# ThomasZiegler/RS-aware-differential-SfM

Hardware: AMD Instinct MI355X
Metric: Mpixels/sec RS depth+pose solve, 1280x720 pair (higher is better)
Workload: dtype f64

## Files before the change

### include/rsdsfm.h

```cpp
#ifndef RSDSFM_H
#define RSDSFM_H

#include <stddef.h>
#include <stdint.h>

#ifdef __cplusplus
extern "C" {
#endif

#define RSDSFM_OK 0
#define RSDSFM_ERR_INVALID (-1)
#define RSDSFM_ERR_HIP (-2)
#define RSDSFM_ERR_NO_DEVICE (-3)
#define RSDSFM_ERR_NUMERIC (-4)
#define RSDSFM_ERR_PENDING (-5)
#define RSDSFM_ERR_PEER (-6)

#define RSDSFM_DEPTH_CLOSED_FORM 0
#define RSDSFM_DEPTH_CERES_LM 1

#define RSDSFM_K_COMPAT 0
#define RSDSFM_K_FIXED 1

#define RSDSFM_FLOW_COMPAT_RANK 0
// ... 110 lines not shown
                                       const double* d_alpha_k_n, int depth_mode, double* d_inv_depth_n);
int rsdsfm_flatten_dev(rsdsfm_ctx* ctx, const double* d_flow_img, int32_t rows, int32_t cols, double fx, double fy,
                       double cx, double cy, double gamma, double flow_threshold, double* d_q2n, double* d_u2n,
                       double* d_alpha_n, double* d_alpha_k_n, int64_t* n_out);
int rsdsfm_depth_map_dev(rsdsfm_ctx* ctx, double* d_inliers_3m_inout, int64_t m, double v_inout[3], double fx, double fy,
                         double cx, double cy, int32_t rows, int32_t cols, double* d_depth_map_colmajor,
                         int32_t* d_xs_or_null, int32_t* d_ys_or_null, int* flipped);
int rsdsfm_pose_table_dev(rsdsfm_ctx* ctx, const double v[3], const double w[3], double k, double gamma, int32_t rows,
                          double* d_R_rows9, double* d_t_rows3);
typedef struct rsdsfm_frame_params {
    int32_t ransac_trials;
    int32_t use_acceleration_mode;
    int32_t use_refinement;
    int32_t depth_mode;
    int32_t k_sign_mode;
    int32_t flow_index_mode;
    int32_t use_global_shutter_mode;
    int32_t struct_bytes;
    double ransac_tol;
    double flow_threshold;
    uint64_t seed;
} rsdsfm_frame_params;

void rsdsfm_frame_params_init(rsdsfm_frame_params* params);

typedef struct rsdsfm_frame_result {
    int64_t n_points, num_inliers;
    int32_t best_trial, flipped;
    double ransac_w[3], ransac_v[3], ransac_k;
    double w[3], v[3], k;
    rsdsfm_lm_summary refine_summary;
    const double* d_inliers;
    const int64_t* d_inlier_idx;
    const int32_t* d_scanline;
} rsdsfm_frame_result;

int rsdsfm_solve_frame_dev(rsdsfm_ctx* ctx, const double* d_flow_img, int32_t rows, int32_t cols, double fx, double fy,
                           double cx, double cy, double gamma, const rsdsfm_frame_params* params,
                           double* d_depth_map_colmajor, double* d_R_rows9_or_null, double* d_t_rows3_or_null,
                           rsdsfm_frame_result* result);
typedef struct rsdsfm_frame_job {
    const double* d_flow_img;
    int32_t rows, cols;
    double fx, fy, cx, cy, gamma;
    double* d_depth_map_colmajor;
    double* d_R_rows9_or_null;
    double* d_t_rows3_or_null;
    uint64_t seed;
} rsdsfm_frame_job;
int rsdsfm_solve_frames_dev(rsdsfm_ctx* ctx, const rsdsfm_frame_job* jobs, int32_t count, const rsdsfm_frame_params* params,
                            rsdsfm_frame_result* results);
int rsdsfm_set_sequence_lanes(rsdsfm_ctx* ctx, int32_t lanes);
int rsdsfm_set_frame_side_flatten(rsdsfm_ctx* ctx, int mode);
int rsdsfm_ransac_dev(rsdsfm_ctx* ctx, const double* d_q2n, const double* d_u2n, const double* d_alpha_n,
                      const double* d_alpha_k_n, int64_t n, int use_alpha_k, int32_t iterations, double tolerance,
                      const int32_t* samples_9xT_or_null, uint64_t seed, int depth_mode, int k_sign_mode,
                      rsdsfm_ransac_out* out);
int rsdsfm_refine_dev(rsdsfm_ctx* ctx, const double* d_flow2n, int64_t n_flow, int64_t m, const double* d_inliers_3m,
                      const double* d_alpha_m, const double* d_alpha_k_m, const int64_t* d_inlier_idx_or_null,
                      const double v_in[3], const double w_in[3], double k_in, int const_acceleration,
                      int flow_index_mode, double* d_inliers_out_3m, double v_out[3], double w_out[3], double* k_out,
                      rsdsfm_lm_summary* summary_or_null);
int rsdsfm_estimate_inverse_depths_batch_dev(rsdsfm_ctx* const* ctxs, int32_t count, const double* const* d_q2n,
                                             const double* const* d_u2n, const int64_t* n, const double* v_count_x3,
                                             const double* w_count_x3, const double* k_count, const double* const* d_alpha_n,
                                             const double* const* d_alpha_k_n, double* const* d_inv_depth_n);
int rsdsfm_depth_lm_batch_launch_dev(rsdsfm_ctx* const* ctxs, int32_t count, const double* const* d_q2n, const double* const* d_u2n,
                                     const int64_t* n, const double* v_count_x3, const double* w_count_x3, const double* k_count,
                                     const double* const* d_alpha_n, const double* const* d_alpha_k_n, double* const* d_inv_depth_n);
int rsdsfm_depth_lm_launch_dev(rsdsfm_ctx* ctx, const double* d_q2n, const double* d_u2n, int64_t n,
                               const double v[3], const double w[3], double k, const double* d_alpha_n,
                               const double* d_alpha_k_n, double* d_inv_depth_n, int launch_id);
int rsdsfm_depth_lm_sums_row_size(void);
int rsdsfm_depth_lm_reduce_dev(rsdsfm_ctx* ctx, int64_t n_shard, double* d_row_out);
int rsdsfm_depth_lm_decide_rows_dev(rsdsfm_ctx* ctx, const double* d_rows, int32_t nrows, int64_t n_total, int launch_id);
int rsdsfm_depth_lm_state(rsdsfm_ctx* ctx, int32_t* status, int32_t* next_launch, rsdsfm_lm_summary* summary_or_null);
int rsdsfm_depth_finish_dev(rsdsfm_ctx* ctx, const double* d_q2n, const double* d_u2n, int64_t n,
                            const double v[3], const double w[3], double k, const double* d_alpha_n,
                            const double* d_alpha_k_n, double* d_inv_depth_n, rsdsfm_lm_summary* summary_or_null,
                            int32_t* extra_launches);

int rsdsfm_flatten_slab_dev(rsdsfm_ctx* ctx, const double* d_img_slab, int32_t rows, int32_t slab_cols, int32_t col0,
                            double fx, double fy, double cx, double cy, double gamma, double thr, double* d_q2n,
                            double* d_u2n, double* d_alpha_n, double* d_alpha_k_n, int64_t* n_out);
int rsdsfm_sample_indices(int64_t n, int32_t iterations, uint64_t seed, int32_t* samples);
int rsdsfm_minimal9_dev(rsdsfm_ctx* ctx, const double* d_q9, const double* d_u9, const double* d_alpha9,
                        const double* d_alpha_k9, int32_t count, int use_alpha_k, int k_sign_mode, double* d_hyp);
int rsdsfm_minimal9_probe_dev(rsdsfm_ctx* ctx, const double* d_q9, const double* d_u9, const double* d_alpha9, const double* d_alpha_k9,
                              int32_t count, int use_alpha_k, int k_sign_mode, int use_cores, double* d_hyp, double* d_probe4);
size_t rsdsfm_tile_lm_state_bytes(void);
size_t rsdsfm_tile_best_bytes(void);
int32_t rsdsfm_tile_ransac_row_size(void);
int32_t rsdsfm_tile_ransac_batch(void);
int rsdsfm_tile_ransac_lm_rows_dev(rsdsfm_ctx* ctx, const double* d_q2n, const double* d_u2n, const double* d_alpha_n,
                                   const double* d_alpha_k_n, int64_t n_shard, const double* d_hyp, int32_t count,
                                   const void* d_states, int32_t round, double tolerance, double* d_rows);
int rsdsfm_tile_ransac_decide_dev(rsdsfm_ctx* ctx, const double* d_rows_all, int32_t nranks, int32_t count, void* d_states,
                                  int64_t n_total, int32_t round, int32_t* d_flags, int32_t* d_scored, double* d_trial_count,
                                  double* d_trial_err);
int rsdsfm_tile_ransac_score_rows_dev(rsdsfm_ctx* ctx, const double* d_q2n, const double* d_u2n, const double* d_alpha_n,
                                      const double* d_alpha_k_n, int64_t n_shard, const double* d_hyp, int32_t count,
                                      const void* d_states, int depth_mode, double tolerance, const int32_t* d_scored_or_null,
                                      double* d_rows);
int rsdsfm_tile_ransac_score_merge_dev(rsdsfm_ctx* ctx, const double* d_rows_all, int32_t nranks, int32_t count,
                                       const int32_t* d_scored_or_null, double* d_trial_count, double* d_trial_err);
int rsdsfm_tile_ransac_pick_dev(rsdsfm_ctx* ctx, const double* d_trial_count, const double* d_trial_err, int32_t iterations,
// ... 105 lines not shown
```

### rs-aware-differential-sfm_amd/__init__.py

```python
import ctypes as C
import os
import sys

import numpy as np

from . import dist, pipeline, synth

_HERE = os.path.dirname(os.path.abspath(__file__))
LIB_PATH = os.environ.get("RSDSFM_LIB") or os.path.join(_HERE, "librsdsfm_hip.so")
LIB_PATH_FUSED = os.path.join(_HERE, "librsdsfm_hip_fused.so")
HEADER_PATH = os.path.join(os.path.dirname(_HERE), "include", "rsdsfm.h")

OK = 0
ERR_PENDING = -5
DEPTH_CLOSED_FORM, DEPTH_CERES_LM = 0, 1
K_COMPAT, K_FIXED = 0, 1
FLOW_COMPAT_RANK, FLOW_GATHERED = 0, 1
REFINE_TRACE_COLS = 8
TRACE_REJECTED, TRACE_ACCEPTED, TRACE_INVALID, TRACE_PARAMETER_TOL, TRACE_FUNCTION_TOL, TRACE_ACCEPTED_GRADIENT_TOL = 0.0, 1.0, 2.0, 3.0, 4.0, 5.0
TERMINATION = {0: "gradient", 1: "parameter", 2: "function", 3: "max_iter", 4: "failure", 5: "min_radius"}

_libs = {}


# ... 439 lines not shown
                              use_acceleration_mode=False, use_refinement=True, depth_mode=DEPTH_CERES_LM, k_sign_mode=K_COMPAT,
                              flow_threshold=1e-10, use_global_shutter_mode=False, flow_index_mode=FLOW_COMPAT_RANK):
        prm = FrameParams(int(trials), int(use_acceleration_mode), int(use_refinement), int(depth_mode), int(k_sign_mode),
                          int(flow_index_mode), int(use_global_shutter_mode), 0, float(tol), float(flow_threshold), int(seed))
        res, info = FrameResult(), TiledInfo()
        d = C.c_double
        self._check(self.lib.rsdsfm_solve_frame_tiled_dev(self._ctx, _dp(d_img_slab) if d_img_slab else None, C.c_int32(rows), C.c_int32(cols), d(K[0]), d(K[1]),
                                                          d(K[2]), d(K[3]), d(gamma), C.byref(prm), _dp(d_depth_map), _dp(d_R) if d_R else None,
                                                          _dp(d_t) if d_t else None, C.byref(res), C.byref(info)), "rsdsfm_solve_frame_tiled_dev")
        return dict(n=int(res.n_points), num_inliers=int(res.num_inliers), best_trial=int(res.best_trial), flipped=bool(res.flipped),
                    ransac_w=np.array(res.ransac_w[:]), ransac_v=np.array(res.ransac_v[:]), ransac_k=float(res.ransac_k),
                    w=np.array(res.w[:]), v=np.array(res.v[:]), k=float(res.k), refine_summary=res.refine_summary.as_dict(),
                    d_inliers=res.d_inliers, d_inlier_idx=res.d_inlier_idx, d_scanline=res.d_scanline, flow_index_mode=int(flow_index_mode),
                    info={k2: int(getattr(info, k2)) for k2, _ in TiledInfo._fields_ if k2 != "_pad"})

    def estimate_inverse_depths_tiled_dev(self, d_q_shard, d_u_shard, n_total, v, w, k, d_alpha_shard, d_alpha_k_shard, d_inv_depth,
                                          mode=DEPTH_CERES_LM):
        sm, info = LmSummary(), TiledInfo()
        opt = lambda p_: _dp(p_) if p_ else None
        self._check(self.lib.rsdsfm_estimate_inverse_depths_tiled_dev(self._ctx, opt(d_q_shard), opt(d_u_shard), C.c_int64(n_total), _v3(v), _v3(w),
                                                                      C.c_double(k), opt(d_alpha_shard), opt(d_alpha_k_shard), C.c_int(int(mode)),
                                                                      opt(d_inv_depth), C.byref(sm), C.byref(info)),
                    "rsdsfm_estimate_inverse_depths_tiled_dev")
        return (sm.as_dict() if int(mode) == DEPTH_CERES_LM else None,
                {k2: int(getattr(info, k2)) for k2, _ in TiledInfo._fields_ if k2 != "_pad"})

    def prepared_frame_solve(self, d_flow_img, rows, cols, K, gamma, d_depth_map, d_R=None, d_t=None, trials=50, tol=0.05,
                             use_acceleration_mode=False, use_refinement=True, depth_mode=DEPTH_CERES_LM, k_sign_mode=K_COMPAT,
                             flow_threshold=1e-10, flow_index_mode=FLOW_COMPAT_RANK, use_global_shutter_mode=False):
        prm = FrameParams(int(trials), int(use_acceleration_mode), int(use_refinement), int(depth_mode), int(k_sign_mode),
                          int(flow_index_mode), int(use_global_shutter_mode), 0, float(tol), float(flow_threshold), 0)
        res = FrameResult()
        d = C.c_double
        fn = self.lib.rsdsfm_solve_frame_dev
        args = (self._ctx, _dp(d_flow_img), C.c_int32(rows), C.c_int32(cols), d(K[0]), d(K[1]), d(K[2]), d(K[3]), d(gamma), C.byref(prm),
                _dp(d_depth_map), _dp(d_R) if d_R else None, _dp(d_t) if d_t else None, C.byref(res))
        check = self._check

        def call(seed):
            prm.seed = seed
            rc = fn(*args)
            if rc != OK:
                check(rc, "rsdsfm_solve_frame_dev")
            return res

        return call

    def set_sequence_lanes(self, lanes):
        self._check(self.lib.rsdsfm_set_sequence_lanes(self._ctx, C.c_int32(int(lanes))), "rsdsfm_set_sequence_lanes")

    def set_frame_side_flatten(self, on):
        self._check(self.lib.rsdsfm_set_frame_side_flatten(self._ctx, int(on)), "rsdsfm_set_frame_side_flatten")

    def prepared_frames_solve(self, jobs, trials=50, tol=0.05, use_acceleration_mode=False, use_refinement=True, depth_mode=DEPTH_CERES_LM,
                              k_sign_mode=K_COMPAT, flow_threshold=1e-10, flow_index_mode=FLOW_COMPAT_RANK, use_global_shutter_mode=False):
        n = len(jobs)
        arr = (FrameJob * n)()
        for a, j in zip(arr, jobs):
            K = j["K"]
            a.d_flow_img, a.rows, a.cols = int(j["d_flow_img"]), int(j["rows"]), int(j["cols"])
            a.fx, a.fy, a.cx, a.cy, a.gamma = float(K[0]), float(K[1]), float(K[2]), float(K[3]), float(j["gamma"])
            a.d_depth_map, a.d_R, a.d_t = int(j["d_depth_map"]), int(j.get("d_R") or 0) or None, int(j.get("d_t") or 0) or None
        prm = FrameParams(int(trials), int(use_acceleration_mode), int(use_refinement), int(depth_mode), int(k_sign_mode),
                          int(flow_index_mode), int(use_global_shutter_mode), 0, float(tol), float(flow_threshold), 0)
        res = (FrameResult * n)()
        fn, ctx, check = self.lib.rsdsfm_solve_frames_dev, self._ctx, self._check

        def call(seeds):
            for a, sd in zip(arr, seeds):
                a.seed = int(sd)
            rc = fn(ctx, arr, C.c_int32(n), C.byref(prm), res)
            if rc != OK:
                check(rc, "rsdsfm_solve_frames_dev")
            return res

        return call

    def solve_frames_dev(self, jobs, seeds, **kw):
        res = self.prepared_frames_solve(jobs, **kw)(seeds)
        return [dict(n=int(r.n_points), num_inliers=int(r.num_inliers), best_trial=int(r.best_trial), flipped=bool(r.flipped),
                     ransac_w=np.array(r.ransac_w[:]), ransac_v=np.array(r.ransac_v[:]), ransac_k=float(r.ransac_k),
                     w=np.array(r.w[:]), v=np.array(r.v[:]), k=float(r.k), refine_summary=r.refine_summary.as_dict(),
                     d_inliers=r.d_inliers, d_inlier_idx=r.d_inlier_idx, d_scanline=r.d_scanline) for r in res]

    def depth_lm_reduce_dev(self, n_shard, d_row):
        self._check(self.lib.rsdsfm_depth_lm_reduce_dev(self._ctx, C.c_int64(n_shard), _dp(d_row)), "rsdsfm_depth_lm_reduce_dev")

    def depth_lm_decide_rows_dev(self, d_rows, nrows, n_total, launch_id):
        self._check(self.lib.rsdsfm_depth_lm_decide_rows_dev(self._ctx, _dp(d_rows), C.c_int32(nrows), C.c_int64(n_total), int(launch_id)), "rsdsfm_depth_lm_decide_rows_dev")

    def depth_lm_state(self):
        status, nxt, sm = C.c_int32(), C.c_int32(), LmSummary()
        self._check(self.lib.rsdsfm_depth_lm_state(self._ctx, C.byref(status), C.byref(nxt), C.byref(sm)), "rsdsfm_depth_lm_state")
        return status.value, nxt.value, sm.as_dict()

    def depth_finish_dev(self, d_q, d_u, n, v, w, k, d_alpha, d_alpha_k, d_rho):
        sm = LmSummary()
        extra = C.c_int32()
        self._check(self.lib.rsdsfm_depth_finish_dev(self._ctx, _dp(d_q), _dp(d_u), C.c_int64(n), _v3(v), _v3(w), C.c_double(k), _dp(d_alpha), _dp(d_alpha_k), _dp(d_rho), C.byref(sm), C.byref(extra)), "rsdsfm_depth_finish_dev")
        return sm.as_dict(), extra.value


def _np0(ptr):
    return _dp(ptr) if ptr else None


# ... 386 lines not shown
```

### rs-aware-differential-sfm_amd/csrc/frame_host.hip

```cpp
#include <stdlib.h>
#include <string.h>

#include <atomic>

#include <algorithm>
#include <new>

#include "rsdsfm_internal.hpp"

namespace rsdsfm {

static std::atomic<int> g_frames_in_flight[64];
int frames_in_flight(const Ctx* c) { return g_frames_in_flight[c->device & 63].load(std::memory_order_relaxed); }

int alpha_ones_launch(Ctx* c, double* d_alpha, int64_t n);
int flatten_device(Ctx* c, const double* d_img, int32_t rows, int32_t cols, int32_t col0, double fx, double fy, double cx, double cy, double gamma,
                   double thr, double* d_q, double* d_u, double* d_alpha, double* d_alpha_k, int64_t* n_out);

struct FrameRun {
    rsdsfm_frame_job job;
    rsdsfm_frame_params prm;
    size_t N = 0;
    int64_t n = 0;
    double *d_q = nullptr, *d_u = nullptr, *d_a = nullptr, *d_ak = nullptr, *d_in_a = nullptr, *d_in_ak = nullptr, *d_inl = nullptr, *d_inl_ref = nullptr;
    int64_t* d_idx = nullptr;
    uint8_t* d_mask = nullptr;
    int32_t* d_ys = nullptr;
    double *d_zpartials = nullptr, *d_zheader = nullptr;
    char* d_refine_ws = nullptr;
    rsdsfm_ransac_out ro;
    RansacRun ransac;
    RefineRun refine;
    Minimal9Direct direct;
    DenseFlatten dense;
    bool refinement_enqueued = false, ahead = false, side_flatten = false, dense_in_launch = false, open = false;
    bool counted = false;
    int rc_begin = RSDSFM_OK;
    int64_t m_known = -1;
    RefineTail tail;
    RansacSpecTail spec_tail;
    std::function<int()> join;
};

namespace {

inline double* header_host(Ctx* c) { return reinterpret_cast<double*>(static_cast<char*>(c->h_pinned) + c->pinned_bytes - 64); }
inline RefineState* state_host(Ctx* c) { return reinterpret_cast<RefineState*>(static_cast<char*>(c->h_pinned) + c->pinned_bytes - kPinnedTail); }
inline int64_t* count_host(Ctx* c) { return reinterpret_cast<int64_t*>(static_cast<char*>(c->h_pinned) + c->pinned_bytes - kPinnedTail / 2); }
static_assert(sizeof(RefineState) + sizeof(int) <= kPinnedTail / 2, "reserved tail: state read-back | point count ... depth-map header");

struct StreamSwap {
    Ctx* c;
    hipStream_t main;
    StreamSwap(Ctx* ctx, hipStream_t other) : c(ctx), main(ctx->stream) { c->stream = other; }
    ~StreamSwap() { c->stream = main; }
};

int ensure_side_stream(Ctx* c) {
    if (c->aux_stream) return RSDSFM_OK;
    RSDSFM_HIP_CHECK(c, hipStreamCreateWithFlags(&c->aux_stream, hipStreamNonBlocking));
    RSDSFM_HIP_CHECK(c, hipEventCreateWithFlags(&c->ev_fork, hipEventDisableTiming));
    RSDSFM_HIP_CHECK(c, hipEventCreateWithFlags(&c->ev_join, hipEventDisableTiming));
    return RSDSFM_OK;
}

static void frame_uncount(const Ctx* c, FrameRun* F) {
    if (F && F->counted) {
        F->counted = false;
        g_frames_in_flight[c->device & 63].fetch_sub(1, std::memory_order_relaxed);
    }
}
struct FrameInFlightEnd {
    const Ctx* c;
    FrameRun* F;
    ~FrameInFlightEnd() { frame_uncount(c, F); }
};

int frame_begin(Ctx* c, FrameRun* F) {
    const rsdsfm_frame_job& J = F->job;
    const rsdsfm_frame_params* prm = &F->prm;
    frame_uncount(c, F);
    F->open = false;
    F->rc_begin = RSDSFM_OK;
    if (J.rows <= 0 || J.cols <= 0 || !J.d_flow_img || !J.d_depth_map_colmajor) return fail(c, RSDSFM_ERR_INVALID, "bad arguments");
    if (prm->flow_index_mode != RSDSFM_FLOW_COMPAT_RANK && prm->flow_index_mode != RSDSFM_FLOW_GATHERED) return fail(c, RSDSFM_ERR_INVALID, "unknown flow_index_mode");
    if (prm->struct_bytes != 0 && prm->struct_bytes != (int32_t)sizeof(rsdsfm_frame_params))
        return fail(c, RSDSFM_ERR_INVALID, "rsdsfm_frame_params: struct_bytes is neither 0 nor sizeof(rsdsfm_frame_params) -- caller built against another header (use rsdsfm_frame_params_init)");
    const int32_t rows = J.rows, cols = J.cols;
    const double fx = J.fx, fy = J.fy, cx = J.cx, cy = J.cy, gamma = J.gamma;
    const size_t N = (size_t)rows * (size_t)cols;
    F->N = N;
    const size_t ncells = (size_t)flatten_cells(rows, cols);
// ... 56 lines not shown
            F->join = [c, F, d_flat_counts, d_flat_offsets]() -> int {
                const rsdsfm_frame_job& J2 = F->job;
                int rc2 = flatten_launch(c, J2.d_flow_img, J2.rows, J2.cols, 0, J2.fx, J2.fy, J2.cx, J2.cy, J2.gamma, F->prm.flow_threshold, F->d_q, F->d_u, F->d_a,
                                         F->d_ak, d_flat_counts, d_flat_offsets, count_host(c), nullptr);
                if (rc2 == RSDSFM_OK && F->prm.use_global_shutter_mode) rc2 = alpha_ones_launch(c, F->d_a, (int64_t)F->N);
                return rc2;
            };
        } else if (side == 1) {
            rc = ensure_side_stream(c);
            if (rc != RSDSFM_OK) return rc;
            RSDSFM_HIP_CHECK(c, hipEventRecord(c->ev_fork, c->stream));
            RSDSFM_HIP_CHECK(c, hipStreamWaitEvent(c->aux_stream, c->ev_fork, 0));
            {
                StreamSwap on_side(c, c->aux_stream);
                rc = flatten_launch(c, J.d_flow_img, rows, cols, 0, fx, fy, cx, cy, gamma, prm->flow_threshold, F->d_q, F->d_u, F->d_a, F->d_ak,
                                    d_flat_counts, d_flat_offsets, count_host(c), nullptr);
                if (rc == RSDSFM_OK && prm->use_global_shutter_mode) rc = alpha_ones_launch(c, F->d_a, n);
            }
            if (rc != RSDSFM_OK) return rc;
            RSDSFM_HIP_CHECK(c, hipEventRecord(c->ev_join, c->aux_stream));
            F->join = [c]() -> int {
                RSDSFM_HIP_CHECK(c, hipStreamWaitEvent(c->stream, c->ev_join, 0));
                return RSDSFM_OK;
            };
        } else {
            rc = flatten_enqueue(c, J.d_flow_img, rows, cols, fx, fy, cx, cy, gamma, prm->flow_threshold, F->d_q, F->d_u, F->d_a, F->d_ak, count_host(c));
            if (rc != RSDSFM_OK) return rc;
        }
    } else {
        rc = flatten_device(c, J.d_flow_img, rows, cols, 0, fx, fy, cx, cy, gamma, prm->flow_threshold, F->d_q, F->d_u, F->d_a, F->d_ak, &n);
        if (rc != RSDSFM_OK) return rc;
        *count_host(c) = n;
    }
    if (prm->use_global_shutter_mode && !F->side_flatten) {
        rc = alpha_ones_launch(c, F->d_a, n);
        if (rc != RSDSFM_OK) return rc;
    }
    F->n = n;
    memset(&F->ro, 0, sizeof(F->ro));
    F->ro.inlier_idx = F->d_idx;
    F->ro.inliers = F->d_inl;
    F->ro.alpha = F->d_in_a;
    F->ro.alpha_k = F->d_in_ak;
    F->ro.mask = F->d_mask;
    F->m_known = -1;
    F->tail = [c, F](const RefineBuffers& B) -> int {
        const rsdsfm_frame_job& J2 = F->job;
        const RefineState* st = B.state;
        const int64_t m_arg = F->m_known >= 0 ? F->m_known : F->n;
        const int64_t* m_dev = F->m_known >= 0 ? nullptr : &st->m;
        PoseTableOut pt;
        if (J2.d_R_rows9_or_null && J2.d_t_rows3_or_null)
            pt.R = J2.d_R_rows9_or_null, pt.t = J2.d_t_rows3_or_null, pt.rows = J2.rows, pt.gamma = J2.gamma, pt.wk_dev = st->p + 3;
        return depth_map_slab_launch(c, F->d_inl_ref, m_arg, F->d_zpartials, refine_finish_grid(c, B), m_arg, nullptr, J2.fx, J2.fy, J2.cx, J2.cy, J2.rows,
                                     0, J2.cols, J2.d_depth_map_colmajor, nullptr, F->d_ys, F->d_zheader, header_host(c), st->p, m_dev, &pt);
    };
    F->spec_tail = [c, F](const RansacBest* d_best) -> int {
        return refine_begin(c, F->d_u, F->n, F->n, F->d_inl, F->d_in_a, F->d_in_ak, F->d_idx, nullptr, nullptr, 0.0, F->prm.use_acceleration_mode,
                            F->prm.flow_index_mode, F->d_inl_ref, &F->tail, d_best, F->d_refine_ws, &F->refine, state_host(c), F->d_zpartials);
    };
    F->refinement_enqueued = false;
    F->ahead = prm->use_refinement && c->ransac_spec_miss < 2;
    F->open = true;
    g_frames_in_flight[c->device & 63].fetch_add(1, std::memory_order_relaxed);
    F->counted = true;
    F->rc_begin = ransac_begin(c, F->d_q, F->d_u, F->d_a, F->d_ak, n, prm->use_acceleration_mode, prm->ransac_trials, prm->ransac_tol, nullptr, J.seed,
                               prm->depth_mode, prm->k_sign_mode, &F->ro, prm->use_refinement ? &F->spec_tail : nullptr, &F->refinement_enqueued, &F->ransac,
                               F->side_flatten ? &F->direct : nullptr, F->side_flatten && !F->dense_in_launch ? &F->join : nullptr,
                               F->dense_in_launch ? &F->dense : nullptr, F->ahead, true);
    return RSDSFM_OK;
}

int frame_finish(Ctx* c, FrameRun* F, rsdsfm_frame_result* res) {
    if (!F->open) return fail(c, RSDSFM_ERR_INVALID, "no frame solve in flight");
    F->open = false;
    FrameInFlightEnd in_flight_end_{c, F};
    const rsdsfm_frame_job& J = F->job;
    const rsdsfm_frame_params* prm = &F->prm;
    memset(res, 0, sizeof(*res));
    int rc = F->rc_begin;
    if (rc == RSDSFM_OK) rc = ransac_finish(c, &F->ransac);
    if (rc != RSDSFM_OK) RSDSFM_HIP_CHECK(c, hipStreamSynchronize(c->stream));
    if (F->side_flatten && c->aux_stream) RSDSFM_HIP_CHECK(c, hipStreamSynchronize(c->aux_stream));
    int64_t n = F->n;
    if (*count_host(c) < 0) {
        c->frame_dense_hint = 1;
        return rc != RSDSFM_OK ? rc : fail(c, RSDSFM_ERR_NUMERIC, "frame solve: the point count did not arrive");
    }
    bool counted = true;
    if (*count_host(c) != n) {
        if (F->dense_in_launch) {
            int64_t n_real = 0;
            rc = flatten_device(c, J.d_flow_img, J.rows, J.cols, 0, J.fx, J.fy, J.cx, J.cy, J.gamma, prm->flow_threshold, F->d_q, F->d_u, F->d_a, F->d_ak, &n_real);
            if (rc == RSDSFM_OK && prm->use_global_shutter_mode) rc = alpha_ones_launch(c, F->d_a, n_real);
            if (rc != RSDSFM_OK) return rc;
            *count_host(c) = n_real;
        }
        n = *count_host(c);
        F->n = n;
        F->refinement_enqueued = false;
        counted = false;
        rc = ransac_begin(c, F->d_q, F->d_u, F->d_a, F->d_ak, n, prm->use_acceleration_mode, prm->ransac_trials, prm->ransac_tol, nullptr, J.seed,
                          prm->depth_mode, prm->k_sign_mode, &F->ro, prm->use_refinement ? &F->spec_tail : nullptr, &F->refinement_enqueued, &F->ransac, nullptr, nullptr,
                          nullptr, F->ahead, true);
        if (rc == RSDSFM_OK) rc = ransac_finish(c, &F->ransac);
        counted = rc == RSDSFM_OK;
    }
    c->frame_dense_hint = n == (int64_t)F->N ? 1 : 0;
    if (rc != RSDSFM_OK) return rc;
    if (counted) ransac_commit_hints(c, F->ransac);
    const rsdsfm_ransac_out& ro = F->ro;
    res->n_points = n;
    res->num_inliers = ro.num_inliers;
    res->best_trial = ro.best_trial;
    memcpy(res->ransac_w, ro.w, sizeof(ro.w));
    memcpy(res->ransac_v, ro.v, sizeof(ro.v));
    res->ransac_k = ro.k;
    double v[3], w[3], k = ro.k;
    for (int i = 0; i < 3; ++i) v[i] = ro.v[i], w[i] = ro.w[i];
    double* d_final = F->d_inl;
    int flipped = 0;
    F->m_known = ro.num_inliers;
    if (prm->use_refinement) {
        bool exact = false;
        if (F->refinement_enqueued) {
            rc = refine_poll(c, &F->refine, v, w, &k, &res->refine_summary);
            exact = rc == kRcRefineRestartExact;
        }
        if (!F->refinement_enqueued || exact)
            rc = refine_device(c, F->d_u, n, ro.num_inliers, F->d_inl, F->d_in_a, F->d_in_ak, F->d_idx, v, w, k, prm->use_acceleration_mode,
                               prm->flow_index_mode, F->d_inl_ref, v, w, &k, &res->refine_summary, &F->tail, F->d_zpartials, exact);
        if (rc != RSDSFM_OK) return rc;
        d_final = F->d_inl_ref;
        const double* h_header = header_host(c);
        flipped = h_header[0] != 0.0;
        v[0] = h_header[1], v[1] = h_header[2], v[2] = h_header[3];
    } else {
        rc = depth_map_device(c, d_final, ro.num_inliers, v, J.fx, J.fy, J.cx, J.cy, J.rows, J.cols, J.d_depth_map_colmajor, nullptr, F->d_ys, &flipped, w,
                              k, J.gamma, J.d_R_rows9_or_null, J.d_t_rows3_or_null);
        if (rc != RSDSFM_OK) return rc;
    }
    res->flipped = flipped;
    memcpy(res->v, v, sizeof(v));
    memcpy(res->w, w, sizeof(w));
    res->k = k;
    res->d_inliers = d_final;
    res->d_inlier_idx = F->d_idx;
    res->d_scanline = F->d_ys;
    return RSDSFM_OK;
}

FrameRun* frame_run_of(Ctx* c) {
    if (!c->frame_run) c->frame_run = new (std::nothrow) FrameRun();
    return static_cast<FrameRun*>(c->frame_run);
}

}

void frame_release(Ctx* c) {
    frame_uncount(c, static_cast<FrameRun*>(c->frame_run));
    delete static_cast<FrameRun*>(c->frame_run);
    c->frame_run = nullptr;
    for (rsdsfm_ctx* lane : c->lanes) rsdsfm_destroy(lane);
    c->lanes.clear();
    if (c->ev_fork) (void)hipEventDestroy(c->ev_fork);
    if (c->ev_join) (void)hipEventDestroy(c->ev_join);
    if (c->ev_seq) (void)hipEventDestroy(c->ev_seq);
    if (c->aux_stream) (void)hipStreamDestroy(c->aux_stream);
    if (c->d_flat_counters) (void)hipFree(c->d_flat_counters);
    c->d_flat_counters = nullptr;
    c->ev_fork = c->ev_join = c->ev_seq = nullptr;
    c->aux_stream = nullptr;
}

}

using namespace rsdsfm;

extern "C" {

void rsdsfm_frame_params_init(rsdsfm_frame_params* p) {
    if (!p) return;
    memset(p, 0, sizeof(*p));
    p->ransac_trials = 5;
    p->use_acceleration_mode = 0;
    p->use_refinement = 1;
    p->depth_mode = RSDSFM_DEPTH_CERES_LM;
    p->k_sign_mode = RSDSFM_K_COMPAT;
    p->flow_index_mode = RSDSFM_FLOW_COMPAT_RANK;
    p->use_global_shutter_mode = 0;
    p->struct_bytes = (int32_t)sizeof(rsdsfm_frame_params);
    p->ransac_tol = 0.05;
    p->flow_threshold = 1e-10;
    p->seed = 1;
}

int rsdsfm_solve_frame_dev(rsdsfm_ctx* ctx, const double* d_flow_img, int32_t rows, int32_t cols, double fx, double fy, double cx,
                           double cy, double gamma, const rsdsfm_frame_params* prm, double* d_depth_map, double* d_R_rows9,
                           double* d_t_rows3, rsdsfm_frame_result* res) {
    if (!ctx) return RSDSFM_ERR_INVALID;
    Ctx* c = &ctx->c;
    DeviceGuard device_guard_(c);
    if (!prm || !res) return fail(c, RSDSFM_ERR_INVALID, "bad arguments");
    FrameRun* F = frame_run_of(c);
    if (!F) return fail(c, RSDSFM_ERR_INVALID, "out of host memory");
    F->prm = *prm;
    F->job = rsdsfm_frame_job{d_flow_img, rows, cols, fx, fy, cx, cy, gamma, d_depth_map, d_R_rows9, d_t_rows3, prm->seed};
    int rc = frame_begin(c, F);
    if (rc != RSDSFM_OK) return rc;
    return frame_finish(c, F, res);
}

int rsdsfm_set_sequence_lanes(rsdsfm_ctx* ctx, int32_t lanes) {
    if (!ctx) return RSDSFM_ERR_INVALID;
    Ctx* c = &ctx->c;
    DeviceGuard device_guard_(c);
    if (lanes < 0 || lanes > 16) return fail(c, RSDSFM_ERR_INVALID, "lanes must be 0 (default) .. 16");
    c->seq_lanes = lanes;
    return RSDSFM_OK;
}

int rsdsfm_set_frame_side_flatten(rsdsfm_ctx* ctx, int mode) {
    if (!ctx) return RSDSFM_ERR_INVALID;
    if (mode < 0 || mode > 3) return fail(&ctx->c, RSDSFM_ERR_INVALID, "mode must be 0 (flatten first), 1 (flatten on a second stream), 2 (flatten behind the minimal solver) or 3 (flatten inside the solver's launch)");
    ctx->c.frame_side_flatten = mode;
    return RSDSFM_OK;
}

int rsdsfm_solve_frames_dev(rsdsfm_ctx* ctx, const rsdsfm_frame_job* jobs, int32_t count, const rsdsfm_frame_params* prm, rsdsfm_frame_result* results) {
    if (!ctx) return RSDSFM_ERR_INVALID;
    Ctx* c = &ctx->c;
    DeviceGuard device_guard_(c);
    if (count < 0 || !prm || (count > 0 && (!jobs || !results))) return fail(c, RSDSFM_ERR_INVALID, "bad arguments");
    if (count == 0) return RSDSFM_OK;
    const int L = std::max(1, std::min<int>(count, c->seq_lanes > 0 ? c->seq_lanes : kSequenceLanesDefault));
    while ((int)c->lanes.size() < L - 1) {
        rsdsfm_ctx* lane = nullptr;
        int rc = rsdsfm_create(&lane, c->device, nullptr);
        if (rc != RSDSFM_OK) return fail(c, rc, "could not create a sequence lane");
        c->lanes.push_back(lane);
    }
    auto lane_ctx = [&](int l) -> Ctx* { return l == 0 ? c : &c->lanes[(size_t)l - 1]->c; };
    if (L > 1) {
        if (!c->ev_seq) RSDSFM_HIP_CHECK(c, hipEventCreateWithFlags(&c->ev_seq, hipEventDisableTiming));
        RSDSFM_HIP_CHECK(c, hipEventRecord(c->ev_seq, c->stream));
    }
    for (int l = 1; l < L; ++l) {
        Ctx* lc = lane_ctx(l);
        RSDSFM_HIP_CHECK(c, hipStreamWaitEvent(lc->stream, c->ev_seq, 0));
        lc->ransac_k0 = c->ransac_k0;
        lc->ransac_math_mode = c->ransac_math_mode;
        lc->lm_arithmetic = c->lm_arithmetic;
        lc->refine_arithmetic = c->refine_arithmetic;
        lc->lma_count_only_force = c->lma_count_only_force;
        lc->frame_side_flatten = c->frame_side_flatten;
        lc->refine_stage_mode = c->refine_stage_mode;
    }
    for (int l = 0; l < L; ++l) lane_ctx(l)->refine_stage_separate = L > 1;
    int first_error = RSDSFM_OK;
    int in_flight[16];
    for (int l = 0; l < 16; ++l) in_flight[l] = -1;
    auto finish_lane = [&](int l) {
        const int i = in_flight[l];
        if (i < 0) return;
        in_flight[l] = -1;
        Ctx* lc = lane_ctx(l);
        int rc = frame_finish(lc, static_cast<FrameRun*>(lc->frame_run), &results[i]);
        if (rc != RSDSFM_OK && first_error == RSDSFM_OK) {
            first_error = rc;
            if (lc != c) c->err = "pair " + std::to_string(i) + ": " + lc->err;
        }
    };
    for (int i = 0; i < count && first_error == RSDSFM_OK; ++i) {
        const int l = i % L;
        finish_lane(l);
        if (first_error != RSDSFM_OK) break;
        Ctx* lc = lane_ctx(l);
        FrameRun* F = frame_run_of(lc);
        if (!F) {
            first_error = fail(c, RSDSFM_ERR_INVALID, "out of host memory");
            break;
        }
        F->prm = *prm;
        F->job = jobs[i];
        int rc = frame_begin(lc, F);
        if (rc != RSDSFM_OK) {
            first_error = rc;
            if (lc != c) c->err = "pair " + std::to_string(i) + ": " + lc->err;
            break;
        }
        in_flight[l] = i;
    }
    for (;;) {
        int best = -1;
        for (int l = 0; l < L; ++l)
            if (in_flight[l] >= 0 && (best < 0 || in_flight[l] < in_flight[best])) best = l;
        if (best < 0) break;
        finish_lane(best);
    }
    for (int l = 0; l < L; ++l) lane_ctx(l)->refine_stage_separate = false;
    return first_error;
}

int rsdsfm_set_refine_stage(rsdsfm_ctx* ctx, int mode) {
    if (!ctx) return RSDSFM_ERR_INVALID;
    Ctx* c = &ctx->c;
    if (mode < 0 || mode > 2) return fail(c, RSDSFM_ERR_INVALID, "refine stage: 0 (automatic), 1 (in the next pass's prologue) or 2 (a launch of its own)");
    c->refine_stage_mode = mode;
// ... 5 lines not shown
```

### rs-aware-differential-sfm_amd/csrc/glue_kernels.hip

```cpp
#include <string.h>

#include <algorithm>

#include "device_math.hpp"
#include "rsdsfm_internal.hpp"

namespace rsdsfm {

__global__ __launch_bounds__(256) void alpha_kernel(const double2* __restrict__ flow_px, int64_t n, double h,
                                                    double gamma, double* __restrict__ alpha) {
    const int64_t stride = (int64_t)gridDim.x * blockDim.x;
    for (int64_t i = (int64_t)blockIdx.x * blockDim.x + threadIdx.x; i < n; i += stride)
        alpha[i] = 1 + gamma * flow_px[i].y / h;
}

__global__ __launch_bounds__(256) void alpha_k_kernel(const double2* __restrict__ q_px, const double2* __restrict__ flow_px,
                                                      int64_t n, double h, double gamma, double* __restrict__ alpha_k) {
    const int64_t stride = (int64_t)gridDim.x * blockDim.x;
    for (int64_t i = (int64_t)blockIdx.x * blockDim.x + threadIdx.x; i < n; i += stride) {
        double y = q_px[i].y, fy = flow_px[i].y;
        double part1 = gamma * y / h;
        double part2 = 1.0 + gamma * (y + fy) / h;
        alpha_k[i] = 0.5 * (part2 * part2 - part1 * part1);
    }
// ... 164 lines not shown
    const double r = wave_sum(acc);
    if ((threadIdx.x & 63) == 0) s_red[threadIdx.x >> 6] = r;
    __syncthreads();
    if (threadIdx.x == 0) {
        const double count_z = ((s_red[0] + s_red[1]) + s_red[2]) + s_red[3];
        const double z_mean = count_z * 1.0 / (double)m;
        const bool flip = z_mean < 0;
        header[0] = flip ? 1.0 : 0.0;
        header[1] = flip ? pose_v.v[0] * -1.0 : pose_v.v[0];
        header[2] = flip ? pose_v.v[1] * -1.0 : pose_v.v[1];
        header[3] = flip ? pose_v.v[2] * -1.0 : pose_v.v[2];
        if (header_host) {
#pragma unroll
            for (int i = 0; i < 4; ++i) header_host[i] = header[i];
        }
        s_v[0] = header[1], s_v[1] = header[2], s_v[2] = header[3];
    }
    if (pt.R) {
        __syncthreads();
        Pose pose;
        pose.v[0] = s_v[0], pose.v[1] = s_v[1], pose.v[2] = s_v[2];
        pose.w[0] = pt.wk_dev[0], pose.w[1] = pt.wk_dev[1], pose.w[2] = pt.wk_dev[2], pose.k = pt.wk_dev[3];
        for (int i = threadIdx.x; i < pt.rows; i += 256) pose_table_row(pose, pt.gamma, pt.rows, i, pt.R, pt.t);
    }
}

__global__ __launch_bounds__(kGB) void depth_claim_kernel(double* __restrict__ inl, int64_t m, const double* __restrict__ header,
                                                         double fx, double fy, double cx, double cy, int rows, int col0,
                                                         int ncols, unsigned* __restrict__ owner, unsigned tag,
                                                         int32_t* __restrict__ xs, int32_t* __restrict__ ys,
                                                         const int64_t* __restrict__ m_dev) {
    if (m_dev) m = *m_dev;
    const bool flip = header[0] != 0.0;
    const int64_t stride = (int64_t)gridDim.x * kGB;
    for (int64_t i = (int64_t)blockIdx.x * kGB + threadIdx.x; i < m; i += stride) {
        if (flip) inl[3 * i + 2] = inl[3 * i + 2] * -1.0;
        const int x = (int)(fx * inl[3 * i] + cx + 0.5);
        const int y = (int)(fy * inl[3 * i + 1] + cy + 0.5);
        if (xs) xs[i] = x;
        if (ys) ys[i] = y;
        if (x >= col0 && x < col0 + ncols && y >= 0 && y < rows) atomicMax(&owner[(int64_t)(x - col0) * rows + y], tag | (unsigned)i);
    }
}

__global__ __launch_bounds__(kGB) void depth_write_kernel(const double* __restrict__ inl, const unsigned* __restrict__ owner, unsigned tag,
                                                         unsigned mask, int64_t npix, double* __restrict__ depth_map) {
    const int64_t stride = (int64_t)gridDim.x * kGB;
    for (int64_t p = (int64_t)blockIdx.x * kGB + threadIdx.x; p < npix; p += stride) {
        const unsigned w = owner[p];
        depth_map[p] = ((w & ~mask) == tag) ? inl[3 * (int64_t)(w & mask) + 2] : 0.0;
    }
}

constexpr int kScanSeg = kScanSegCells;

__global__ __launch_bounds__(256) void cell_scan_local_kernel(const int64_t* __restrict__ counts, int64_t ncells,
                                                             int64_t* __restrict__ offsets, int64_t* __restrict__ seg_totals) {
    __shared__ int s_cnt[kScanSeg];
    __shared__ int s_wave[4];
    const int tid = threadIdx.x, lane = tid & 63, wv = tid >> 6;
    const int64_t base = (int64_t)blockIdx.x * kScanSeg;
#pragma unroll
    for (int k = 0; k < kScanSeg / 256; ++k) {
        const int64_t i = base + k * 256 + tid;
        s_cnt[k * 256 + tid] = i < ncells ? (int)counts[i] : 0;
    }
    __syncthreads();
    int v[kScanSeg / 256];
    int sum = 0;
#pragma unroll
    for (int k = 0; k < kScanSeg / 256; ++k) {
        v[k] = s_cnt[tid * (kScanSeg / 256) + k];
        sum += v[k];
    }
    int incl = sum;
    for (int off = 1; off < 64; off <<= 1) {
        const int o = __shfl_up(incl, off, 64);
        if (lane >= off) incl += o;
    }
    if (lane == 63) s_wave[wv] = incl;
    __syncthreads();
    int wbase = 0;
    for (int w2 = 0; w2 < wv; ++w2) wbase += s_wave[w2];
    int run = wbase + incl - sum;
#pragma unroll
    for (int k = 0; k < kScanSeg / 256; ++k) {
        const int64_t i = base + (int64_t)tid * (kScanSeg / 256) + k;
        if (i < ncells) offsets[i] = run;
        run += v[k];
    }
    if (tid == 255) seg_totals[blockIdx.x] = run;
}

__global__ __launch_bounds__(256) void cell_scan_segments_kernel(int64_t* __restrict__ seg_totals, int nseg, int64_t* __restrict__ total) {
    __shared__ int64_t s_part[256];
    const int tid = threadIdx.x;
    const int per = (nseg + 255) / 256;
    int64_t sum = 0;
    for (int j = 0; j < per; ++j) {
        const int b = tid * per + j;
        if (b < nseg) sum += seg_totals[b];
    }
    s_part[tid] = sum;
    __syncthreads();
    if (tid == 0) {
        int64_t run = 0;
// ... 50 lines not shown
    hipLaunchKernelGGL(flatten_tile_kernel<1>, grid, dim3(kGB), 0, c->stream, img2, rows, cols, fx, fy, cx, cy, gamma, thr, col0, nchunks,
                       d_counts, d_offsets, d_seg, reinterpret_cast<double2*>(d_q), reinterpret_cast<double2*>(d_u), d_alpha, d_alpha_k, 0,
                       (int64_t*)nullptr);
    RSDSFM_HIP_CHECK(c, hipGetLastError());
    return RSDSFM_OK;
}

__global__ __launch_bounds__(256) void zsum_row_kernel(const double* __restrict__ partials, int nblocks, double* __restrict__ out) {
    __shared__ double s_red[4];
    double acc = 0.0;
    for (int b = threadIdx.x; b < nblocks; b += 256) acc += partials[b];
    const double r = wave_sum(acc);
    if ((threadIdx.x & 63) == 0) s_red[threadIdx.x >> 6] = r;
    __syncthreads();
    if (threadIdx.x == 0) out[0] = ((s_red[0] + s_red[1]) + s_red[2]) + s_red[3];
}

static inline int zsum_blocks(int64_t m) { return (int)std::min<int64_t>(1024, std::max<int64_t>(1, (m + kGB - 1) / kGB)); }

int zsum_row_launch(Ctx* c, const double* d_inl, int64_t m, double* d_partials, double* d_out) {
    const int zb = zsum_blocks(m);
    hipLaunchKernelGGL(zsum_partial_kernel, dim3(zb), dim3(kGB), 0, c->stream, d_inl, m, d_partials, (const int64_t*)nullptr);
    RSDSFM_HIP_CHECK(c, hipGetLastError());
    hipLaunchKernelGGL(zsum_row_kernel, dim3(1), dim3(256), 0, c->stream, d_partials, zb, d_out);
    RSDSFM_HIP_CHECK(c, hipGetLastError());
    return RSDSFM_OK;
}

int depth_map_slab_launch(Ctx* c, double* d_inl, int64_t m, const double* d_zsums, int nz, int64_t m_total, const double v[3],
                          double fx, double fy, double cx, double cy, int rows, int col0, int ncols, double* d_depth_map,
                          int32_t* d_xs, int32_t* d_ys, double* d_header, double* h_header, const double* v_dev, const int64_t* m_dev,
                          const PoseTableOut* pt) {
    const int64_t npix = (int64_t)rows * ncols;
    if (m >= ((int64_t)1 << 31)) return fail(c, RSDSFM_ERR_INVALID, "depth map: more than 2^31 inliers");
    Pose pv;
    memset(&pv, 0, sizeof(pv));
    if (v) pv.v[0] = v[0], pv.v[1] = v[1], pv.v[2] = v[2];
    hipLaunchKernelGGL(zsum_decide_kernel, dim3(1), dim3(256), 0, c->stream, d_zsums, nz, m_total, pv, d_header, h_header, v_dev, m_dev,
                       pt ? *pt : PoseTableOut());
    RSDSFM_HIP_CHECK(c, hipGetLastError());
    unsigned *d_owner = nullptr, tag = 0, mask = 0;
    int rc = claim_map_acquire(c, 2, (size_t)std::max<int64_t>(std::max<int64_t>(npix, m), 1), &d_owner, &tag, &mask);
    if (rc != RSDSFM_OK) return rc;
    if (m > 0) {
        hipLaunchKernelGGL(depth_claim_kernel, dim3(stream_grid(m)), dim3(kGB), 0, c->stream, d_inl, m, d_header, fx, fy, cx, cy, rows,
                           col0, ncols, d_owner, tag, d_xs, d_ys, m_dev);
        RSDSFM_HIP_CHECK(c, hipGetLastError());
    }
    hipLaunchKernelGGL(depth_write_kernel, dim3(stream_grid(npix)), dim3(kGB), 0, c->stream, d_inl, d_owner, tag, mask, npix, d_depth_map);
    RSDSFM_HIP_CHECK(c, hipGetLastError());
    return RSDSFM_OK;
}

int depth_map_launch(Ctx* c, double* d_inl, int64_t m, const double v[3], double fx, double fy, double cx, double cy, int rows,
                     int cols, double* d_depth_map, int32_t* d_xs, int32_t* d_ys, double* d_header, double* d_partials,
                     double* h_header, const double* v_dev, const int64_t* m_dev, const PoseTableOut* pt) {
    const int zb = zsum_blocks(m);
    hipLaunchKernelGGL(zsum_partial_kernel, dim3(zb), dim3(kGB), 0, c->stream, d_inl, m, d_partials, m_dev);
    RSDSFM_HIP_CHECK(c, hipGetLastError());
    return depth_map_slab_launch(c, d_inl, m, d_partials, zb, m, v, fx, fy, cx, cy, rows, 0, cols, d_depth_map, d_xs, d_ys, d_header,
                                 h_header, v_dev, m_dev, pt);
}

}
```

### rs-aware-differential-sfm_amd/csrc/ransac_host.hip

```cpp
#include <stdio.h>
#include <stdlib.h>
#include <string.h>

#include <algorithm>
#include <vector>

#include "rsdsfm_internal.hpp"

namespace rsdsfm {

namespace {


inline uint64_t splitmix64(uint64_t& state) {
    uint64_t z = (state += 0x9E3779B97F4A7C15ULL);
    z = (z ^ (z >> 30)) * 0xBF58476D1CE4E5B9ULL;
    z = (z ^ (z >> 27)) * 0x94D049BB133111EBULL;
    return z ^ (z >> 31);
}

void sample_indices(int64_t n, int T, uint64_t seed, std::vector<int32_t>& out) {
    struct Slot {
        int64_t key;
        int32_t val;
// ... 106 lines not shown
                }
                R.b0 = 0;
                R.pc = kPcBatchBegin;
                break;
            }
            case kPcBatchBegin: {
                if (R.b0 >= T) {
                    R.pc = kPcFinal;
                    break;
                }
                R.B = std::min(batch, T - R.b0);
                R.need_score = true;
                if (depth_mode == RSDSFM_DEPTH_CERES_LM) {
                    if (R.b0 > 0)
                        RSDSFM_HIP_CHECK(c, hipMemsetAsync(R.d_flags, 0, (size_t)(reinterpret_cast<char*>(R.d_irr_count + R.batch) - reinterpret_cast<char*>(R.d_flags)), c->stream));
                    R.round = 0;
                    R.pc = kPcRoundEnqueue;
                } else {
                    R.pc = kPcScore;
                }
                break;
            }
            case kPcRoundEnqueue: {
                const int b0 = R.b0, B = R.B, round = R.round;
                bool flags_via_pick = false;
                if (round > 4 * kMaxIter) return fail(c, RSDSFM_ERR_NUMERIC, "LM state machines did not terminate");
                if (R.analytic && round == 0) {
                    rc = ransac_lma_launch(c, R.d_q, R.d_u, R.d_a, R.d_ak, n, R.d_hyp + (size_t)b0 * 8, B, R.d_states + b0, R.d_partials, R.d_flags,
                                           R.d_scored + b0, R.d_tcount + b0, R.d_terr + b0, tol, R.lma_cand, 2, R.d_irr_count, R.d_irr_list, R.d_unscored,
                                           nullptr, R.core_epoch ? c->d_core_flag : nullptr, R.core_epoch, R.count_only);
                } else {
                    rc = ransac_lm_round_launch(c, R.d_q, R.d_u, R.d_a, R.d_ak, n, R.d_hyp + (size_t)b0 * 8, B, R.d_states + b0, R.d_partials, R.d_flags,
                                                R.d_scored + b0, R.d_tcount + b0, R.d_terr + b0, round, tol, R.k0, R.fused_base, R.core_math,
                                                R.core_epoch ? c->d_core_flag : nullptr, R.core_epoch, R.d_unscored);
                }
                if (rc != RSDSFM_OK) return rc;
                if (round == 0 && B == T) {
                    const PickLazy lazy = R.count_only ? PickLazy{R.d_scored, R.d_unscored, R.d_flags + 1} : PickLazy();
                    if (c->ransac_score_idle < kScoreIdleLimit) {
                        if (R.count_only) {
                            rc = ransac_pick_launch(c, R.d_tcount, R.d_terr, T, R.d_hyp, R.d_best, nullptr, R.d_flags, nullptr, 0, nullptr, 0, 0, nullptr, 0.0, lazy);
                            if (rc != RSDSFM_OK) return rc;
                        }
                        rc = ransac_score_launch(c, R.d_q, R.d_u, R.d_a, R.d_ak, n, R.d_hyp, T, R.d_states, depth_mode, tol, R.d_scored, R.d_partials,
                                                 R.d_tcount, R.d_terr, R.d_unscored, R.d_flags + 1);
                        if (rc != RSDSFM_OK) return rc;
                        R.spec_scored = true;
                    }
                    rc = ransac_pick_launch(c, R.d_tcount, R.d_terr, T, R.d_hyp, R.d_best, R.h_best, R.d_flags, R.h_running, R.spec_scored ? 1 : 0,
                                            nullptr, 0, 0, nullptr, R.tie_margin, lazy);
                    if (rc != RSDSFM_OK) return rc;
                    flags_via_pick = true;
                    rc = ransac_final_launch(c, R.d_q, R.d_u, R.d_a, R.d_ak, n, R.d_best, R.d_states, depth_mode, tol, R.d_rho, R.d_mask, R.d_bcounts,
                                             R.d_boffs, out->inlier_idx, out->inliers, out->alpha, out->alpha_k, R.h_best);
                    if (rc != RSDSFM_OK) return rc;
                    R.final_done = true;
                    R.spec_final = true;
                    if (R.spec_tail && R.tail_ahead) {
                        rc = (*R.spec_tail)(R.d_best);
                        if (rc != RSDSFM_OK) return rc;
                        R.tail_enqueued = true;
                    }
                }
                if (!flags_via_pick) RSDSFM_HIP_CHECK(c, hipMemcpyAsync(R.h_running, R.d_flags, sizeof(int) * 8, hipMemcpyDeviceToHost, c->stream));
                R.pc = kPcRoundWait;
                if (yield_at_wait) return RSDSFM_OK;
                break;
            }
            case kPcRoundWait: {
                yield_at_wait = false;
                if (int rcs = sync_stream(c, "ransac_finish line 244")) return rcs;
                const int* h_running = R.h_running;
                if (R.round == 0 && R.analytic && (h_running[3] & 16) != 0) R.lma_guard |= h_running[3] >> 8;
                if (R.round == 0 && R.analytic && (h_running[3] & 6) != 0 && !((h_running[3] & 1) && R.core_math)) {
                    rc = lma_start_over(c, R, (h_running[3] >> 8) | ((h_running[3] & 4) ? (1 << 7) : 0));
                    if (rc != RSDSFM_OK) return rc;
                    break;
                }
                if (R.round == 0 && R.core_math && (h_running[3] & 1) != 0) {
                    R.core_math = false;
                    R.restarted = true;
                    R.not_one_step = 0;
                    R.final_done = R.spec_scored = R.tail_enqueued = R.spec_final = false;
                    R.dense = nullptr;
                    R.after_minimal9 = nullptr;
                    R.pc = kPcStart;
                    break;
                }
                if (R.round == 0) {
                    R.not_one_step += h_running[2];
                    if (R.b0 == 0) {
                        int best = 0;
                        for (int a2 = 1; a2 <= 3; ++a2)
                            if (h_running[4 + a2] > (best ? h_running[4 + best] : 0)) best = a2;
                        if (best) R.fused_base_next = best;
                        int second = 0;
                        for (int a2 = 1; a2 <= 3; ++a2)
                            if (a2 != best && h_running[4 + a2] > (second ? h_running[4 + second] : 0)) second = a2;
                        if (best) {
                            R.lma_cand_next[0] = best;
                            R.lma_cand_next[1] = second ? second : (best > 1 ? best - 1 : 2);
                        }
                    }
                }
                if (h_running[0] == 0) {
                    R.pc = kPcAfterRounds;
                } else {
                    R.final_done = false;
                    R.round += 1;
                    R.pc = kPcRoundEnqueue;
                }
                break;
            }
            case kPcAfterRounds: {
                R.need_score = R.h_running[1] > 0;
                if (R.B == T) R.score_hint_next = R.need_score ? 1 : 0;
                if (R.need_score && R.final_done && R.spec_scored && !R.h_best->lazy_pending) R.need_score = false;
                if (R.need_score) R.final_done = false;
                R.pc = kPcScore;
                break;
            }
            case kPcScore: {
                if (R.need_score) {
                    rc = ransac_score_launch(c, R.d_q, R.d_u, R.d_a, R.d_ak, n, R.d_hyp + (size_t)R.b0 * 8, R.B, R.d_states + R.b0, depth_mode, tol,
                                             depth_mode == RSDSFM_DEPTH_CERES_LM ? R.d_scored + R.b0 : nullptr, R.d_partials, R.d_tcount + R.b0,
                                             R.d_terr + R.b0, depth_mode == RSDSFM_DEPTH_CERES_LM ? R.d_unscored : nullptr, R.d_flags + 1);
                    if (rc != RSDSFM_OK) return rc;
                }
                R.b0 += batch;
                R.pc = kPcBatchBegin;
                break;
            }
            case kPcFinal: {
                if (!R.final_done) {
                    R.tail_enqueued = false;
                    R.spec_final = false;
                    rc = ransac_pick_launch(c, R.d_tcount, R.d_terr, T, R.d_hyp, R.d_best, R.h_best, nullptr, nullptr, 0, nullptr, 0, 0, nullptr, R.tie_margin,
                                            R.count_only ? PickLazy{R.d_scored, R.d_unscored, R.d_flags + 1} : PickLazy());
                    if (rc != RSDSFM_OK) return rc;
                    rc = ransac_final_launch(c, R.d_q, R.d_u, R.d_a, R.d_ak, n, R.d_best, R.d_states, depth_mode, tol, R.d_rho, R.d_mask, R.d_bcounts,
                                             R.d_boffs, out->inlier_idx, out->inliers, out->alpha, out->alpha_k, R.h_best);
                    if (rc != RSDSFM_OK) return rc;
                }
                if (R.spec_tail && !R.tail_enqueued) {
                    rc = (*R.spec_tail)(R.d_best);
                    if (rc != RSDSFM_OK) return rc;
                    R.tail_enqueued = true;
                }
                if (T > 0 && out->trial_count) RSDSFM_HIP_CHECK(c, hipMemcpyAsync(R.h_tcount, R.d_tcount, sizeof(double) * T, hipMemcpyDeviceToHost, c->stream));
                if (T > 0 && out->trial_err) RSDSFM_HIP_CHECK(c, hipMemcpyAsync(R.h_terr, R.d_terr, sizeof(double) * T, hipMemcpyDeviceToHost, c->stream));
                if (T > 0 && out->trial_vel) RSDSFM_HIP_CHECK(c, hipMemcpyAsync(R.h_hyp, R.d_hyp, sizeof(double) * 8 * T, hipMemcpyDeviceToHost, c->stream));
                if (T > 0 && out->trial_steps && depth_mode == RSDSFM_DEPTH_CERES_LM)
                    RSDSFM_HIP_CHECK(c, hipMemcpyAsync(R.h_states, R.d_states, sizeof(LmState) * T, hipMemcpyDeviceToHost, c->stream));
                R.pc = kPcFinalWait;
                if (yield_at_wait) return RSDSFM_OK;
                break;
            }
            case kPcFinalWait: {
                if (int rcs = sync_stream(c, "ransac_finish line 345")) return rcs;
                const RansacBest* h_best = R.h_best;
#ifdef RSDSFM_DEBUG_HOOKS
                if (getenv("RSDSFM_RANSAC_DEBUG")) fprintf(stderr, "[ransac] final wait: lazy_pending %d undecided %d flags %d %d %d %d hist %d %d %d %d spec_scored %d spec_final %d tail %d idle %d\n", h_best->lazy_pending, h_best->undecided, R.h_running[0], R.h_running[1], R.h_running[2], R.h_running[3], R.h_running[4], R.h_running[5], R.h_running[6], R.h_running[7], (int)R.spec_scored, (int)R.spec_final, (int)R.tail_enqueued, c->ransac_score_idle);
#endif
                if (R.count_only && h_best->lazy_pending) {
                    if (++R.lazy_rounds > T + 2) return fail(c, RSDSFM_ERR_NUMERIC, "lazy error sums did not settle");
                    R.final_done = R.tail_enqueued = R.spec_final = false;
                    R.need_score = true;
                    R.score_hint_next = 1;
                    R.b0 = 0;
                    R.B = T;
                    R.pc = kPcScore;
                    break;
                }
                if (R.analytic && h_best->lma_tie) {
                    rc = lma_start_over(c, R, 1 << 7);
                    if (rc != RSDSFM_OK) return rc;
                    break;
                }
                R.lma_tie_seen = h_best->lma_tie != 0;
                R.shared_best = h_best->shared_best;
                if (h_best->num_inliers != h_best->num_inliers_scan) {
                    if (R.analytic) {
                        rc = lma_start_over(c, R, 1 << 10);
                        if (rc != RSDSFM_OK) return rc;
                        break;
                    }
                    return fail(c, RSDSFM_ERR_NUMERIC, "inlier count mismatch between scoring and compaction");
                }
                out->num_inliers = h_best->num_inliers;
                out->best_trial = h_best->best_trial;
                memcpy(out->w, &h_best->hyp[0], 3 * sizeof(double));
                memcpy(out->v, &h_best->hyp[3], 3 * sizeof(double));
                out->k = h_best->hyp[6];
                out->inlier_error = h_best->inlier_error;
                for (int t = 0; t < T; ++t) {
                    if (out->trial_count) out->trial_count[t] = (int64_t)R.h_tcount[t];
                    if (out->trial_err) out->trial_err[t] = R.h_terr[t];
                    if (out->trial_vel) memcpy(out->trial_vel + (size_t)7 * t, R.h_hyp + (size_t)8 * t, 7 * sizeof(double));
                    if (out->trial_steps) out->trial_steps[t] = depth_mode == RSDSFM_DEPTH_CERES_LM ? R.h_states[t].num_successful : 1;
                }
                if (R.spec_tail_held) *R.spec_tail_held = R.tail_enqueued;
                R.hints_ready = true;
                R.pc = kPcDone;
                (void)Tn;
                return RSDSFM_OK;
            }
            default:
                return RSDSFM_OK;
        }
    }
}

}

void ransac_commit_hints(Ctx* c, const RansacRun& R) {
    if (!R.hints_ready || R.depth_mode != RSDSFM_DEPTH_CERES_LM || R.T <= 0) return;
    if (R.fused_base_next) c->ransac_fused_base = R.fused_base_next;
    if (R.score_hint_next >= 0) c->ransac_score_idle = R.score_hint_next ? 0 : std::min(c->ransac_score_idle + 1, kScoreIdleLimit);
    c->ransac_not_one_step = R.not_one_step;
    c->ransac_spec_miss = R.spec_final ? 0 : std::min(c->ransac_spec_miss + 1, 2);
    if (R.count_only) c->lma_count_only_runs += 1, c->lma_lazy_runs += (R.lazy_rounds > 0 || R.shared_best > 1) ? 1 : 0;
    if (R.lazy_rounds > 0 || R.shared_best > 1) c->lma_unique_run = 0;
    else if (R.shared_best == 1) c->lma_unique_run = std::min(c->lma_unique_run + 1, 2);
    if (R.lma_guard) c->lma_last_guard = R.lma_guard, c->lma_handed_over += 1;
    if (R.lma_restarted) {
        c->lma_hold = 16;
        c->lma_restarts += 1;
        c->lma_last_guard = R.lma_guard;
    } else if (c->lma_hold > 0 && !R.analytic) {
        c->lma_hold = R.lma_tie_seen ? 16 : c->lma_hold - 1;
    }
    if (R.restarted) {
        c->ransac_standard_math = 16;
        c->ransac_restarts += 1;
    } else if (c->ransac_standard_math > 0) {
        c->ransac_standard_math -= 1;
    }
}

int ransac_begin(Ctx* c, const double* d_q, const double* d_u, const double* d_a, const double* d_ak, int64_t n, int use_alpha_k, int T,
                 double tol, const int32_t* h_samples, uint64_t seed, int depth_mode, int k_sign_mode, rsdsfm_ransac_out* out,
                 const RansacSpecTail* spec_tail, bool* spec_tail_held, RansacRun* run, const Minimal9Direct* direct,
                 const std::function<int()>* after_minimal9, const DenseFlatten* dense, bool tail_ahead, bool count_only) {
    RansacRun& R = *run;
    R = RansacRun();
    R.tail_ahead = tail_ahead;
    R.core_math = c->ransac_math_mode == 0 && c->ransac_standard_math == 0;
    R.analytic = depth_mode == RSDSFM_DEPTH_CERES_LM && T > 0 && c->lm_arithmetic == 0 && c->lma_hold == 0;
    R.tie_margin = depth_mode != RSDSFM_DEPTH_CERES_LM || c->lm_arithmetic != 0 ? 0.0 : (R.analytic ? kLmaTie : -kLmaTie);
    R.lma_cand[0] = c->lma_cand[0], R.lma_cand[1] = c->lma_cand[1];
    R.count_only = count_only && R.analytic && T <= kRansacBatch && (c->lma_unique_run >= 2 || c->lma_count_only_force);
    if (R.count_only) R.tie_margin = 0.0;
    if (spec_tail_held) *spec_tail_held = false;
    if (!out) return fail(c, RSDSFM_ERR_INVALID, "null out");
    if (n < 9) return fail(c, RSDSFM_ERR_INVALID, "ransac needs at least 9 points (the reference would compute rand() % 0)");
    if (T < 0) return fail(c, RSDSFM_ERR_INVALID, "negative iterations");
    if (depth_mode != RSDSFM_DEPTH_CLOSED_FORM && depth_mode != RSDSFM_DEPTH_CERES_LM) return fail(c, RSDSFM_ERR_INVALID, "unknown depth_mode");
    if (n > (int64_t)INT32_MAX) return fail(c, RSDSFM_ERR_INVALID, "n exceeds the int32 sample index range");
    if (T > 0) {
        if (h_samples) {
            R.samples.assign(h_samples, h_samples + (size_t)T * 9);
            for (int32_t s : R.samples)
                if (s < 0 || s >= n) return fail(c, RSDSFM_ERR_INVALID, "sample index out of range");
        } else {
            sample_indices(n, T, seed, R.samples);
        }
    }
    const int Tn = std::max(T, 1);
    const int batch = std::min(Tn, kRansacBatch);
    const size_t partials_doubles = std::max<size_t>((size_t)ransac_lm_partials_doubles(c, n, batch), (size_t)ransac_lma_partials_doubles(c, n, batch));
    size_t need = Arena::need(sizeof(double) * Tn * 8) + Arena::need(sizeof(int) * batch) + Arena::need(sizeof(int) * ransac_lma_list_ints(batch)) +
                  Arena::need(sizeof(LmState) * Tn) + Arena::need(sizeof(double) * partials_doubles) +
                  Arena::need(sizeof(int) * 8) + 2 * Arena::need(sizeof(int) * Tn) + 2 * Arena::need(sizeof(double) * Tn) + Arena::need(sizeof(RansacBest)) +
                  2 * Arena::need(sizeof(int64_t) * 2048) + Arena::need(sizeof(double) * (size_t)n) + Arena::need((size_t)n) + 4096;
    int rc = ensure_ws(c, need);
    if (rc != RSDSFM_OK) return rc;
    Arena ws(c->d_ws);
    R.d_hyp = ws.take<double>((size_t)Tn * 8);
    R.zero_begin = ws.base + ws.off;
    R.d_states = ws.take<LmState>(Tn);
    R.d_scored = ws.take<int>(Tn);
    R.d_flags = ws.take<int>(8);
    R.d_irr_count = ws.take<int>(batch);
    R.zero_bytes = (size_t)((ws.base + ws.off) - R.zero_begin);
    R.d_irr_list = ws.take<int>(ransac_lma_list_ints(batch));
    R.d_unscored = ws.take<int>(batch);
    R.d_partials = ws.take<double>(partials_doubles);
    R.d_tcount = ws.take<double>(Tn);
    R.d_terr = ws.take<double>(Tn);
    R.d_best = ws.take<RansacBest>(1);
    R.d_bcounts = ws.take<int64_t>(2048);
    R.d_boffs = ws.take<int64_t>(2048);
    R.d_rho = out->inv_depth ? out->inv_depth : ws.take<double>((size_t)n);
    R.d_mask = out->mask ? out->mask : ws.take<uint8_t>((size_t)n);

    rc = ensure_pinned(c, ransac_pinned_bytes(T));
    if (rc != RSDSFM_OK) return rc;
    if (!c->d_core_flag) {
        RSDSFM_HIP_CHECK(c, hipMalloc(reinterpret_cast<void**>(&c->d_core_flag), 64));
        RSDSFM_HIP_CHECK(c, hipMemsetAsync(c->d_core_flag, 0, 64, c->stream));
    }
    char* hp = static_cast<char*>(c->h_pinned);
    R.h_best = reinterpret_cast<RansacBest*>(hp);
    R.h_running = reinterpret_cast<int*>(hp + sizeof(RansacBest));
    R.h_tcount = reinterpret_cast<double*>(hp + sizeof(RansacBest) + 32);
// ... 148 lines not shown
```

### rs-aware-differential-sfm_amd/csrc/ransac_kernels.hip

```cpp
#include <algorithm>

#include "device_math.hpp"
#include "lm_common.hpp"
#include "rsdsfm_internal.hpp"

namespace rsdsfm {

namespace {

constexpr int kRB = 256;
constexpr int kRP = RSDSFM_FUSED ? 5 : 6;
constexpr int kFused = 1;
constexpr int kTiledFusedBase = 2;
constexpr int NSR = NS + 2 * kFused;
constexpr int kNSum = NSR - (KMAX + 1);
constexpr int kTStride = 65;

template <int K0>
struct R0Shape {
    static constexpr int NSk = 3 + 5 * K0;
    static constexpr int F = kFused;
    static constexpr int nsum = NSk - (K0 + 1) + 2 * F;
};
static_assert(R0Shape<KMAX>::nsum == kNSum, "full shape uses every sum slot");
// ... 713 lines not shown
        }
        rho_out[i] = rho;
        mask_out[i] = in ? 1 : 0;
        count += in ? 1 : 0;
    }
    for (int off = 32; off >= 1; off >>= 1) count += __shfl_xor(count, off, 64);
    if (lane == 0) s_cnt[wv] = count;
    __syncthreads();
    if (tid == 0) {
        int c = 0;
        for (int w2 = 0; w2 < kRB / 64; ++w2) c += s_cnt[w2];
        block_counts[blockIdx.x] = c;
    }
}

__global__ __launch_bounds__(256) void ransac_scan_kernel(const int64_t* __restrict__ block_counts, int nblocks,
                                                         int64_t* __restrict__ block_offsets, RansacBest* best, RansacBest* best_host) {
    __shared__ int64_t s_part[256];
    const int tid = threadIdx.x;
    const int per = (nblocks + 255) / 256;
    int64_t sum = 0;
    for (int j = 0; j < per; ++j) {
        const int b = tid * per + j;
        if (b < nblocks) sum += block_counts[b];
    }
    s_part[tid] = sum;
    __syncthreads();
    if (tid == 0) {
        int64_t run = 0;
        for (int i = 0; i < 256; ++i) {
            int64_t v = s_part[i];
            s_part[i] = run;
            run += v;
        }
        best->num_inliers_scan = run;
        if (best_host) best_host->num_inliers_scan = run;
    }
    __syncthreads();
    int64_t run = s_part[tid];
    for (int j = 0; j < per; ++j) {
        const int b = tid * per + j;
        if (b < nblocks) {
            block_offsets[b] = run;
            run += block_counts[b];
        }
    }
}

__global__ __launch_bounds__(kRB) void ransac_scatter_kernel(const double2* __restrict__ q, const double* __restrict__ alpha,
                                                            const double* __restrict__ alpha_k, int64_t n, int64_t chunk,
                                                            const double* __restrict__ rho, const uint8_t* __restrict__ mask,
                                                            const int64_t* __restrict__ block_counts, RansacBest* best,
                                                            RansacBest* best_host, int64_t* __restrict__ inlier_idx, double* __restrict__ inliers,
                                                            double* __restrict__ out_alpha, double* __restrict__ out_alpha_k) {
    __shared__ int s_wave[kRB / 64];
    __shared__ int64_t s_base;
    __shared__ int64_t s_pre[kRB / 64], s_all[kRB / 64];
    const int tid = threadIdx.x, lane = tid & 63, wv = tid >> 6;
    const int undecided = best->undecided;
    const int64_t i0 = (int64_t)blockIdx.x * chunk;
    const int64_t i1 = (i0 + chunk < n) ? i0 + chunk : n;
    {
        int64_t pre = 0, all = 0;
        for (int b = tid; b < (int)gridDim.x; b += kRB) {
            const int64_t cnt = block_counts[b];
            all += cnt;
            if (b < (int)blockIdx.x) pre += cnt;
        }
#pragma unroll
        for (int off = 32; off > 0; off >>= 1) {
            pre += __shfl_down(pre, off);
            all += __shfl_down(all, off);
        }
        if (lane == 0) s_pre[wv] = pre, s_all[wv] = all;
        __syncthreads();
        if (tid == 0) {
            int64_t p2 = 0, a2 = 0;
            for (int w2 = 0; w2 < kRB / 64; ++w2) p2 += s_pre[w2], a2 += s_all[w2];
            s_base = p2;
            if (blockIdx.x == 0 && !undecided) {
                best->num_inliers_scan = a2;
                if (best_host) best_host->num_inliers_scan = a2;
            }
        }
    }
    if (undecided) return;
    __syncthreads();
    for (int64_t start = i0; start < i1; start += kRB) {
        const int64_t i = start + tid;
        const bool in = (i < i1) && mask[i] != 0;
        const unsigned long long bal = __ballot(in);
        const int prefix = __popcll(bal & ((1ull << lane) - 1ull));
        if (lane == 0) s_wave[wv] = __popcll(bal);
        __syncthreads();
        int woff = 0, total = 0;
#pragma unroll
        for (int w2 = 0; w2 < kRB / 64; ++w2) {
            const int c = s_wave[w2];
            if (w2 < wv) woff += c;
            total += c;
        }
        if (in) {
            const int64_t o = s_base + woff + prefix;
            double2 qq = q[i];
            if (inlier_idx) inlier_idx[o] = i;
            if (inliers) {
                inliers[3 * o + 0] = qq.x;
                inliers[3 * o + 1] = qq.y;
                inliers[3 * o + 2] = 1.0 / rho[i];
// ... 119 lines not shown
    return RSDSFM_OK;
}

int ransac_rows_payload_doubles(int T, bool core_trailer) { return T * NSR + (core_trailer ? 2 : 0); }

int ransac_decide_rows_launch(Ctx* c, const double* rows_all, int nranks, int T, LmState* states, int64_t n_total, int round,
                              int* flags, int* scored, double* trial_count, double* trial_err, bool core_trailer, double* cnt_rt, int cnt_stride) {
    if (cnt_rt && nranks > 256) return fail(c, RSDSFM_ERR_INVALID, "more than 256 ranks");
    RSDSFM_HIP_CHECK(c, hipMemsetAsync(flags, 0, sizeof(int), c->stream));
    hipLaunchKernelGGL(ransac_decide_kernel, dim3(T), dim3(256), 0, c->stream, rows_all, nranks, T, 0, states, n_total, round, (int)KMAX, flags,
                       static_cast<int*>(nullptr), scored, trial_count, trial_err, kTiledFusedBase, static_cast<int*>(nullptr),
                       static_cast<int*>(nullptr), core_trailer ? T * NSR / 2 + 1 : 0, cnt_rt, cnt_stride);
    RSDSFM_HIP_CHECK(c, hipGetLastError());
    return RSDSFM_OK;
}

int ransac_score_rows_launch(Ctx* c, const double* q, const double* u, const double* a, const double* ak, int64_t n,
                             const double* hyp, int T, const LmState* states, int depth_mode, double tol, const int* scored,
                             double* partials, double* rows) {
    const int grid = ransac_pixel_grid(c, n);
    const int groups = ransac_lm_groups(c, grid, T);
    hipLaunchKernelGGL(ransac_score_kernel, dim3(((grid + 7) / 8) * 8 * groups), dim3(kRB), sizeof(double) * T * 2, c->stream,
                       reinterpret_cast<const double2*>(q), reinterpret_cast<const double2*>(u), a, ak, n, hyp, T, states,
                       depth_mode, tol, scored, partials, grid, groups, static_cast<const int*>(nullptr), static_cast<const int*>(nullptr));
    RSDSFM_HIP_CHECK(c, hipGetLastError());
    hipLaunchKernelGGL(ransac_score_rows_kernel, dim3(T), dim3(256), 0, c->stream, partials, grid, T, scored, rows);
    RSDSFM_HIP_CHECK(c, hipGetLastError());
    return RSDSFM_OK;
}

int ransac_score_merge_launch(Ctx* c, const double* rows_all, int nranks, int T, const int* scored, double* trial_count,
                              double* trial_err, double* cnt_rt, int cnt_stride) {
    if (cnt_rt && nranks > 256) return fail(c, RSDSFM_ERR_INVALID, "more than 256 ranks");
    hipLaunchKernelGGL(ransac_reduce_scores_kernel, dim3(T), dim3(256), 0, c->stream, rows_all, nranks, T, scored, trial_count,
                       trial_err, cnt_rt, cnt_stride);
    RSDSFM_HIP_CHECK(c, hipGetLastError());
    return RSDSFM_OK;
}

int ransac_rows_doubles() { return NSR; }

int ransac_pick_launch(Ctx* c, const double* trial_count, const double* trial_err, int T, const double* hyp, RansacBest* best,
                       RansacBest* best_host, const int* d_flags, int* h_flags, int scored_ahead, const double* cnt_rt, int cnt_stride,
                       int nranks, int64_t* m_all, double tie_margin, PickLazy lazy) {
    hipLaunchKernelGGL(ransac_pick_kernel, dim3(1), dim3(64), 0, c->stream, trial_count, trial_err, T, hyp, best, best_host, d_flags, h_flags, scored_ahead,
                       cnt_rt, cnt_stride, nranks, m_all, tie_margin, lazy);
    RSDSFM_HIP_CHECK(c, hipGetLastError());
    return RSDSFM_OK;
}

int ransac_final_launch(Ctx* c, const double* q, const double* u, const double* a, const double* ak, int64_t n,
                        RansacBest* best, const LmState* states, int depth_mode, double tol, double* rho, uint8_t* mask,
                        int64_t* block_counts, int64_t* block_offsets, int64_t* inlier_idx, double* inliers,
                        double* out_alpha, double* out_alpha_k, RansacBest* best_host) {
    int64_t blocks = (n + kRB - 1) / kRB;
    if (blocks < 1) blocks = 1;
    const int64_t cap = 2048;
    int64_t chunk = kRB;
    if (blocks > cap) {
        chunk = ((blocks + cap - 1) / cap) * kRB;
        blocks = (n + chunk - 1) / chunk;
    }
    hipLaunchKernelGGL(ransac_final_kernel, dim3((int)blocks), dim3(kRB), 0, c->stream, reinterpret_cast<const double2*>(q),
                       reinterpret_cast<const double2*>(u), a, ak, n, chunk, best, states, depth_mode, tol, rho, mask,
                       block_counts);
    RSDSFM_HIP_CHECK(c, hipGetLastError());
    if (inlier_idx || inliers || out_alpha || out_alpha_k) {
        hipLaunchKernelGGL(ransac_scatter_kernel, dim3((int)blocks), dim3(kRB), 0, c->stream, reinterpret_cast<const double2*>(q),
                           a, ak, n, chunk, rho, mask, block_counts, best, best_host, inlier_idx, inliers, out_alpha, out_alpha_k);
    } else {
        hipLaunchKernelGGL(ransac_scan_kernel, dim3(1), dim3(256), 0, c->stream, block_counts, (int)blocks, block_offsets, best, best_host);
    }
    RSDSFM_HIP_CHECK(c, hipGetLastError());
    return RSDSFM_OK;
}

}
```

### rs-aware-differential-sfm_amd/csrc/refine_host.hip

```cpp
#include <string.h>

#include <algorithm>

#include "rsdsfm_internal.hpp"

namespace rsdsfm {

int refine_begin(Ctx* c, const double* d_flow, int64_t n_flow, int64_t m, const double* d_inl, const double* d_alpha,
                 const double* d_alpha_k, const int64_t* d_inlier_idx, const double v_in[3], const double w_in[3], double k_in,
                 int const_acceleration, int flow_index_mode, double* d_inl_out, const RefineTail* tail, const RansacBest* d_best,
                 void* ws_base, RefineRun* run, RefineState* hs_prefetch, double* d_zpartials, bool exact) {
    if (m < 0 || n_flow < 0 || (!d_best && (!v_in || !w_in))) return fail(c, RSDSFM_ERR_INVALID, "bad arguments");
    if (flow_index_mode != RSDSFM_FLOW_COMPAT_RANK && flow_index_mode != RSDSFM_FLOW_GATHERED) return fail(c, RSDSFM_ERR_INVALID, "unknown flow_index_mode");
    if (flow_index_mode == RSDSFM_FLOW_GATHERED && m > 0 && !d_inlier_idx) return fail(c, RSDSFM_ERR_INVALID, "gathered mode needs inlier_idx");
    if (m > 0 && (!d_flow || !d_inl || !d_alpha || !d_alpha_k || !d_inl_out)) return fail(c, RSDSFM_ERR_INVALID, "null device pointer");
    const int np = const_acceleration ? 7 : 6;
    const size_t M = (size_t)std::max<int64_t>(m, 1);
    const size_t npart = (size_t)(d_best ? refine_partials_doubles_cap(c) : refine_partials_doubles(c, m));
    int rc = RSDSFM_OK;
    if (!ws_base) {
        rc = ensure_ws(c, refine_workspace_bytes(c, m, d_best != nullptr));
        if (rc != RSDSFM_OK) return rc;
        ws_base = c->d_ws;
    }
    rc = ensure_pinned(c, sizeof(RefineState) + 64);
    if (rc != RSDSFM_OK) return rc;
    Arena ws(ws_base);
    RefineBuffers& B = run->B;
    B = RefineBuffers();
    B.flow = d_flow;
    B.n_flow = n_flow;
    B.m = m;
    B.m_on_device = d_best != nullptr;
    B.inl = d_inl;
    B.alpha = d_alpha;
    B.alpha_k = d_alpha_k;
    B.inlier_idx = d_inlier_idx;
    B.flow_index_mode = flow_index_mode;
    static_assert(sizeof(RefineState) % sizeof(int) == 0, "flag follows the state");
    char* state_block = ws.take<char>(sizeof(RefineState) + 64);
    B.state = reinterpret_cast<RefineState*>(state_block);
    B.uu = ws.take<double>(4 * M);
    B.beta = ws.take<double>(M);
    B.rho_a = ws.take<double>(M);
    B.rho_b = ws.take<double>(M);
    B.srho = ws.take<double>(M);
    B.partials = ws.take<double>(npart);
    B.bad_index = reinterpret_cast<int*>(state_block + sizeof(RefineState));
    B.zpartials = d_zpartials;
    run->np = np;
    run->rf = !exact && c->lm_arithmetic == 0 && c->refine_arithmetic == 0;
    if (run->rf) c->refine_rf_runs += 1;
    run->d_inl_out = d_inl_out;
    run->tail = tail;
    run->launched = 0;
    run->hint_prev = c->refine_iters_hint;
    run->hs = hs_prefetch ? hs_prefetch : static_cast<RefineState*>(c->h_pinned);
    run->prefetch = hs_prefetch != nullptr;
    run->prefetched = false;
    B.state_host = hs_prefetch;
    if (d_best) {
        rc = refine_state_from_best_launch(c, d_best, B, np);
        if (rc != RSDSFM_OK) return rc;
    } else {
        RefineState* hs = static_cast<RefineState*>(c->h_pinned);
        int* h_bad = reinterpret_cast<int*>(static_cast<char*>(c->h_pinned) + sizeof(RefineState));
        memset(hs, 0, sizeof(RefineState));
        hs->np = np;
        for (int i = 0; i < 3; ++i) {
            hs->p[i] = v_in[i];
            hs->p[3 + i] = w_in[i];
        }
        hs->p[6] = k_in;
        hs->termination = -1;
        hs->radius = kInitialRadius;
        hs->need_schur = 1;
        memset(h_bad, 0, kRefineStateBlockTail);
        RSDSFM_HIP_CHECK(c, hipMemcpyAsync(B.state, hs, sizeof(RefineState) + kRefineStateBlockTail, hipMemcpyHostToDevice, c->stream));
    }
    rc = refine_trace_reset(c);
    if (rc != RSDSFM_OK) return rc;
    if (!run->rf) {
        rc = refine_init_launch(c, B, np);
        if (rc != RSDSFM_OK) return rc;
    }
    const int hp = run->hint_prev;
    run->chunk = (hp >= 0 && hp <= 3) ? hp + 1 : (hp > 8 ? std::min(hp + 1, 28) : 7);
    return refine_enqueue_chunk(c, run);
}

int refine_enqueue_chunk(Ctx* c, RefineRun* run) {
    static const bool watch = getenv("RSDSFM_SYNC_WATCHDOG_S") != nullptr;
    if (watch) {
        const RefineBuffers B = run->B;
        const int launched = run->launched, chunk = run->chunk, rf = run->rf ? 1 : 0;
        set_sync_dumper([B, launched, chunk, rf](Ctx* cc) {
            fprintf(stderr, "[rsdsfm] last refinement chunk enqueued: slots [%d, %d), radius-factorised %d\n", launched, launched + chunk, rf);
            refine_rf_debug_dump(cc, B);
        });
    }
    if (run->rf) {
        for (int i = 0; i <= run->chunk; ++i) {
            const int g = run->launched + i;
            int rc = refine_rf_pass_launch(c, run->B, run->np, g, run->launched, nullptr, 0, -1, nullptr, i == run->chunk);
            if (rc != RSDSFM_OK) return rc;
        }
        run->launched += 1;
    } else {
        for (int i = 0; i < run->chunk; ++i) {
            int rc = refine_iter_launch(c, run->B, run->np, i, run->chunk);
            if (rc != RSDSFM_OK) return rc;
        }
    }
    run->launched += run->chunk;
    int rc = refine_finish_launch(c, run->B, run->d_inl_out);
    if (rc != RSDSFM_OK) return rc;
    run->tail_done = false;
    if (run->tail && !(run->hint_prev > run->launched + 1)) {
        rc = (*run->tail)(run->B);
        run->tail_done = true;
    }
    if (rc != RSDSFM_OK) return rc;
    if (run->prefetch) run->prefetched = true;
    return rc;
}

int refine_poll(Ctx* c, RefineRun* run, double v_out[3], double w_out[3], double* k_out, rsdsfm_lm_summary* summary) {
    if (!v_out || !w_out || !k_out) return fail(c, RSDSFM_ERR_INVALID, "bad arguments");
    RefineState* hs = run->hs;
    int* h_bad = reinterpret_cast<int*>(reinterpret_cast<char*>(hs) + sizeof(RefineState));
    for (bool first = true;; first = false) {
        if (!(first && run->prefetch && run->prefetched)) {
            if (!run->prefetch) RSDSFM_HIP_CHECK(c, hipMemcpyAsync(hs, run->B.state, sizeof(RefineState) + sizeof(int), hipMemcpyDeviceToHost, c->stream));
            if (int rcs = sync_stream(c, "refine_poll line 168")) return rcs;
        }
        if (*h_bad) return fail(c, RSDSFM_ERR_INVALID, "flow index out of range (flow has fewer columns than inliers / bad inlier_idx)");
        if (hs->termination == kTermRestartExact) {
            c->refine_rf_restarts += 1;
            c->refine_rf_last_guard = hs->rf_guard;
            return kRcRefineRestartExact;
        }
        if (hs->termination >= 0) {
            if (run->tail && !run->tail_done) {
                int rc = (*run->tail)(run->B);
                if (rc != RSDSFM_OK) return rc;
                run->tail_done = true;
                if (int rcs = sync_stream(c, "refine_poll line 181")) return rcs;
            }
            break;
        }
        if (run->launched > 8 * kMaxIter + 16) return fail(c, RSDSFM_ERR_NUMERIC, "refinement did not terminate");
        run->chunk = std::min(8, std::max(2, run->hint_prev - run->launched));
        int rc = refine_enqueue_chunk(c, run);
        if (rc != RSDSFM_OK) return rc;
    }
    c->refine_iters_hint = hs->slots;
    if (run->rf) c->refine_rf_resolves += hs->rf_resolves;
    for (int i = 0; i < 3; ++i) {
        v_out[i] = hs->p[i];
        w_out[i] = hs->p[3 + i];
    }
    *k_out = hs->p[6];
    if (summary) {
        summary->num_iterations = hs->iteration;
        summary->num_successful_steps = hs->num_successful;
        summary->num_unsuccessful_steps = hs->num_unsuccessful;
        summary->termination = hs->termination;
        summary->initial_cost = hs->initial_cost;
        summary->final_cost = hs->cost;
        summary->final_radius = hs->radius;
    }
    return RSDSFM_OK;
}

size_t refine_workspace_bytes(const Ctx* c, int64_t m, bool m_on_device) {
    const size_t M = (size_t)std::max<int64_t>(m, 1);
    const size_t npart = (size_t)(m_on_device ? refine_partials_doubles_cap(c) : refine_partials_doubles(c, m));
    return Arena::need(sizeof(RefineState) + 64) + Arena::need(32 * M) + 4 * Arena::need(8 * M) + Arena::need(8 * npart) + Arena::need(64) + 1024;
}

int refine_device(Ctx* c, const double* d_flow, int64_t n_flow, int64_t m, const double* d_inl, const double* d_alpha,
                  const double* d_alpha_k, const int64_t* d_inlier_idx, const double v_in[3], const double w_in[3], double k_in,
                  int const_acceleration, int flow_index_mode, double* d_inl_out, double v_out[3], double w_out[3], double* k_out,
                  rsdsfm_lm_summary* summary, const RefineTail* tail, double* d_zpartials, bool exact) {
    if (!v_out || !w_out || !k_out) return fail(c, RSDSFM_ERR_INVALID, "bad arguments");
    const double v0[3] = {v_in[0], v_in[1], v_in[2]}, w0[3] = {w_in[0], w_in[1], w_in[2]};
    for (int attempt = 0;; ++attempt) {
        RefineRun run;
        int rc = refine_begin(c, d_flow, n_flow, m, d_inl, d_alpha, d_alpha_k, d_inlier_idx, v0, w0, k_in, const_acceleration, flow_index_mode,
                              d_inl_out, tail, nullptr, nullptr, &run, nullptr, d_zpartials, exact || attempt > 0);
        if (rc != RSDSFM_OK) return rc;
        rc = refine_poll(c, &run, v_out, w_out, k_out, summary);
        if (rc != kRcRefineRestartExact || attempt > 0) return rc == kRcRefineRestartExact ? fail(c, RSDSFM_ERR_NUMERIC, "refinement: restart loop") : rc;
    }
}

}

using namespace rsdsfm;

extern "C" {

int rsdsfm_refine_dev(rsdsfm_ctx* ctx, const double* d_flow, int64_t n_flow, int64_t m, const double* d_inl, const double* d_alpha,
                      const double* d_alpha_k, const int64_t* d_inlier_idx, const double v_in[3], const double w_in[3], double k_in,
                      int const_acceleration, int flow_index_mode, double* d_inl_out, double v_out[3], double w_out[3], double* k_out,
                      rsdsfm_lm_summary* summary) {
    if (!ctx) return RSDSFM_ERR_INVALID;
    DeviceGuard device_guard_(&ctx->c);
    return refine_device(&ctx->c, d_flow, n_flow, m, d_inl, d_alpha, d_alpha_k, d_inlier_idx, v_in, w_in, k_in, const_acceleration,
                         flow_index_mode, d_inl_out, v_out, w_out, k_out, summary, nullptr, nullptr);
}

static int refine_host(rsdsfm_ctx* ctx, uint64_t tag, const double* flow, int64_t n_flow, int64_t m, const double* inl, const double* alpha,
                       const double* alpha_k, const int64_t* inlier_idx, const double v_in[3], const double w_in[3], double k_in,
                       int const_acceleration, int flow_index_mode, double* inl_out, double v_out[3], double w_out[3], double* k_out,
                       rsdsfm_lm_summary* summary) {
    if (!ctx) return RSDSFM_ERR_INVALID;
    Ctx* c = &ctx->c;
    DeviceGuard device_guard_(c);
    if (m < 0 || n_flow < 0) return fail(c, RSDSFM_ERR_INVALID, "bad arguments");
    if (m > 0 && (!flow || !inl || !alpha || !alpha_k || !inl_out)) return fail(c, RSDSFM_ERR_INVALID, "null pointer");
    const size_t M = (size_t)m, NF = (size_t)n_flow;
    const Ctx::RansacCache& rcache = c->ransac_cache;
    bool cached = tag != 0 && tag == rcache.tag && rcache.stage_gen == c->stage_gen && rcache.m == m && M > 0 && (inlier_idx != nullptr || flow_index_mode == RSDSFM_FLOW_COMPAT_RANK);
    for (int j = 0; cached && j < 16; ++j) cached = memcmp(&rcache.inl_probe[j], &inl[(3 * M - 1) * (size_t)j / 15], sizeof(double)) == 0;
    bool flow_cached = cached && flow == rcache.h_u && n_flow == rcache.n;
    for (int j = 0; flow_cached && j < 16; ++j) flow_cached = memcmp(&rcache.u_probe[j], &flow[(2 * NF - 1) * (size_t)j / 15], sizeof(double)) == 0;
    int rc = RSDSFM_OK;
    const double *d_flow, *d_inl, *d_a, *d_ak;
    const int64_t* d_idx;
    double* d_out;
    if (cached) {
        const size_t extra = Arena::need(24 * M) + (flow_cached ? 0 : Arena::need(16 * NF)) + 1024;
        const size_t ws_ref = refine_workspace_bytes(c, m, false);
        rc = ensure_ws(c, ws_ref + extra);
        if (rc != RSDSFM_OK) return rc;
        Arena xa(static_cast<char*>(c->d_ws) + ((ws_ref + 255) & ~(size_t)255));
        d_out = xa.take<double>(3 * M);
        double* d_fl = flow_cached ? nullptr : xa.take<double>(2 * NF);
        if (!flow_cached && NF && (rc = xfer_h2d(c, d_fl, flow, 16 * NF)) != RSDSFM_OK) return rc;
        d_flow = flow_cached ? rcache.d_u : d_fl;
        d_inl = rcache.d_inl, d_a = rcache.d_alpha, d_ak = rcache.d_alpha_k, d_idx = inlier_idx ? rcache.d_idx : nullptr;
        c->refine_cache_hits += 1;
// ... 51 lines not shown
```

### rs-aware-differential-sfm_amd/csrc/refine_kernels.hip

```cpp
#include "refine_common.hpp"

namespace rsdsfm {


template <int NP>
__global__ __launch_bounds__(kFB) void refine_init_kernel(const double2* __restrict__ flow, int64_t n_flow, int64_t m,
                                                         const double* __restrict__ inl, const double* __restrict__ alpha,
                                                         const double* __restrict__ alpha_k,
                                                         const int64_t* __restrict__ inlier_idx, int flow_index_mode,
                                                         const RefineState* __restrict__ st, double4* __restrict__ xyuv,
                                                         double* __restrict__ beta_out, double* __restrict__ rho0,
                                                         double* __restrict__ srho, double* __restrict__ partials,
                                                         int* __restrict__ bad_index, int want_zsum) {
    using CT = Counts<NP>;
    __shared__ double s_red[kFB / 64][CT::NINIT];
    const PassShape ps = pass_shape(st, m);
    if (!ps.live) return;
    m = ps.m;
    double p[7];
#pragma unroll
    for (int c = 0; c < 7; ++c) p[c] = st->p[c];
    double acc[CT::NINIT];
#pragma unroll
    for (int s = 0; s < CT::NINIT; ++s) acc[s] = 0.0;
// ... 378 lines not shown
        if (tr) tr[7] = RSDSFM_TRACE_REJECTED;
        st->num_unsuccessful += 1;
        st->radius = st->radius / st->decrease_factor;
        st->decrease_factor *= 2.0;
    }
    return st->termination < 0 && st->num_successful > successful_before ? 1 : 0;
}

template <int NP>
__global__ __launch_bounds__(kFB) void refine_decide_kernel(const double* __restrict__ partials, int nblocks,
                                                           RefineState* st, double* __restrict__ trace, int trace_rows) {
    using CT = Counts<NP>;
    __shared__ double s_red[kFB / 64][CT::NBACK];
    __shared__ double s[CT::NBACK];
    if (st->termination >= 0) return;
    const int solve_ok = st->solve_ok;
    if (solve_ok) reduce_partials<CT::NBACK>(partials, nblocks >= 0 ? nblocks : st->grid, CT::BACK_MAX, s_red, s);
    if (threadIdx.x != 0) return;
    (void)decide_serial<NP>(st, s, solve_ok, trace, trace_rows);
}

__global__ __launch_bounds__(kFB) void refine_finish_kernel(int64_t m, const double* __restrict__ inl,
                                                           const double* __restrict__ rho_a, const double* __restrict__ rho_b,
                                                           const RefineState* __restrict__ st, double* __restrict__ inl_out,
                                                           double* __restrict__ zpartials, RefineState* __restrict__ state_host,
                                                           const int* __restrict__ bad_index) {
    __shared__ double s_red[kFB / 64];
    if (state_host && blockIdx.x == 0) {
        static_assert(sizeof(RefineState) % 8 == 0, "copied as 8-byte words");
        for (int i = threadIdx.x; i < (int)(sizeof(RefineState) / 8); i += kFB)
            reinterpret_cast<double*>(state_host)[i] = reinterpret_cast<const double*>(st)[i];
        if (threadIdx.x == 0) *reinterpret_cast<int*>(reinterpret_cast<char*>(state_host) + sizeof(RefineState)) = *bad_index;
    }
    const double* __restrict__ rho = st->cur ? rho_b : rho_a;
    if (m < 0) m = st->m;
    const int64_t stride = (int64_t)gridDim.x * kFB;
    double acc = 0.0;
    for (int64_t i = (int64_t)blockIdx.x * kFB + threadIdx.x; i < m; i += stride) {
        inl_out[3 * i] = inl[3 * i];
        inl_out[3 * i + 1] = inl[3 * i + 1];
        const double z = 1.0 / rho[i];
        inl_out[3 * i + 2] = z;
        acc += z;
    }
    if (zpartials) {
        const double r = wave_sum(acc);
        if ((threadIdx.x & 63) == 0) s_red[threadIdx.x >> 6] = r;
        __syncthreads();
        if (threadIdx.x == 0) {
            double t = s_red[0];
            for (int w2 = 1; w2 < kFB / 64; ++w2) t += s_red[w2];
            zpartials[blockIdx.x] = t;
        }
    }
}

__global__ void refine_state_from_best_kernel(const RansacBest* __restrict__ best, RefineState* __restrict__ st, int np, int cap,
                                              int* __restrict__ bad_index) {
    if (threadIdx.x != 0 || blockIdx.x != 0) return;
    RefineState z;
    memset(&z, 0, sizeof(z));
    z.np = np;
    for (int i = 0; i < 3; ++i) {
        z.p[i] = best->hyp[3 + i];
        z.p[3 + i] = best->hyp[i];
    }
    z.p[6] = best->hyp[6];
    z.termination = -1;
    z.radius = kInitialRadius;
    z.need_schur = 1;
    const int64_t m = best->undecided ? 0 : best->num_inliers_scan;
    z.m = m;
    int64_t b = (m + kFB - 1) / kFB;
    if (b < 1) b = 1;
    if (b > cap) {
        const int64_t iters = (b + cap - 1) / cap;
        b = (b + iters - 1) / iters;
    }
    z.grid = (int)b;
    *st = z;
    bad_index[0] = 0;
    bad_index[4] = bad_index[5] = bad_index[6] = 0;
}

static inline int refine_grid_cap(const Ctx* c) { return c->num_cus * kWorkgroupsPerCu; }
static inline int refine_grid(const Ctx* c, int64_t m) {
    int64_t b = (m + kFB - 1) / kFB;
    const int64_t cap = (int64_t)c->num_cus * kWorkgroupsPerCu;
    if (b < 1) b = 1;
    if (b > cap) {
        const int64_t iters = (b + cap - 1) / cap;
        b = (b + iters - 1) / iters;
    }
    return (int)b;
}

static inline int refine_partials_half(const Ctx* c) { return refine_grid_cap(c) * SlotRow<7>::NW; }
constexpr int kStateDoubles = (int)((sizeof(RefineState) + 63) / 64 * 8);
int refine_partials_doubles_cap(const Ctx* c) { return 2 * refine_partials_half(c) + 2 * kStateDoubles + 8 + refine_rf_extra_doubles(); }
int refine_partials_half_doubles(const Ctx* c) { return refine_partials_half(c); }
int refine_state_doubles() { return kStateDoubles; }
int refine_partials_doubles(const Ctx* c, int64_t m) { (void)m; return refine_partials_doubles_cap(c); }
static inline double* rows_buffer(const Ctx* c, const RefineBuffers& B, int which) { return B.partials + (size_t)(which & 1) * refine_partials_half(c); }
static inline RefineState* chunk_state(const Ctx* c, const RefineBuffers& B, int which) {
    return reinterpret_cast<RefineState*>(B.partials + 2 * (size_t)refine_partials_half(c) + (size_t)(which & 1) * kStateDoubles);
}
// ... 297 lines not shown
                           j == chunk - 1 ? B.state : chunk_state(c, B, j), c->d_refine_trace, c->refine_trace_rows);
        RSDSFM_HIP_CHECK(c, hipGetLastError());
    }
    return RSDSFM_OK;
}

template <int NP>
static int refine_slot_rows_t(Ctx* c, const RefineBuffers& B, double* row, int j, const double* rows_all_prev, int nranks) {
    const int grid = B.m_on_device ? refine_grid_cap(c) : refine_grid(c, B.m);
    hipLaunchKernelGGL(refine_slot_pass_kernel<NP>, dim3(grid), dim3(kFB), 0, c->stream, B.m_on_device ? (int64_t)-1 : B.m, reinterpret_cast<const double4*>(B.uu), B.beta, B.alpha,
                       B.alpha_k, B.rho_a, B.rho_b, B.srho, slot_state_in(c, B, j), chunk_state(c, B, j), rows_all_prev, nranks, rows_buffer(c, B, 0),
                       B.want_zsum ? 1 : 0, c->d_refine_trace, c->refine_trace_rows);
    RSDSFM_HIP_CHECK(c, hipGetLastError());
    hipLaunchKernelGGL(refine_slot_row_kernel<NP>, dim3(1), dim3(kFB), 0, c->stream, rows_buffer(c, B, 0), B.m_on_device ? -1 : grid, row,
                       static_cast<const RefineState*>(B.state));
    RSDSFM_HIP_CHECK(c, hipGetLastError());
    return RSDSFM_OK;
}
int refine_slot_row_doubles(int np) { return np == 7 ? SlotRow<7>::NW : SlotRow<6>::NW; }
int refine_slot_partials_doubles(const Ctx* c, int64_t m) { return refine_partials_doubles(c, m); }
int refine_slot_rows_launch(Ctx* c, const RefineBuffers& B, int np, double* row, int j, const double* rows_all_prev, int nranks) {
    return np == 7 ? refine_slot_rows_t<7>(c, B, row, j, rows_all_prev, nranks) : refine_slot_rows_t<6>(c, B, row, j, rows_all_prev, nranks);
}
int refine_slot_apply_launch(Ctx* c, const RefineBuffers& B, int np, const double* rows_all, int nranks, int chunk) {
    if (np == 7)
        hipLaunchKernelGGL(refine_slot_apply_kernel<7>, dim3(1), dim3(kFB), 0, c->stream, rows_all, nranks, chunk_state(c, B, chunk - 1), B.state,
                           c->d_refine_trace, c->refine_trace_rows);
    else
        hipLaunchKernelGGL(refine_slot_apply_kernel<6>, dim3(1), dim3(kFB), 0, c->stream, rows_all, nranks, chunk_state(c, B, chunk - 1), B.state,
                           c->d_refine_trace, c->refine_trace_rows);
    RSDSFM_HIP_CHECK(c, hipGetLastError());
    return RSDSFM_OK;
}

int refine_stage_row_doubles(int np, int stage) {
    if (np == 7) return stage == 0 ? Counts<7>::NINIT : stage == 1 ? Counts<7>::NSCHUR : Counts<7>::NBACK;
    return stage == 0 ? Counts<6>::NINIT : stage == 1 ? Counts<6>::NSCHUR : Counts<6>::NBACK;
}
int refine_stage_rows_launch(Ctx* c, const RefineBuffers& B, int np, int stage, double* row) {
    return np == 7 ? refine_stage_rows_t<7>(c, B, stage, row) : refine_stage_rows_t<6>(c, B, stage, row);
}
int refine_stage_apply_launch(Ctx* c, const RefineBuffers& B, int np, int stage, const double* rows_all, int nranks, int64_t m_total, const int64_t* m_total_dev) {
    return np == 7 ? refine_stage_apply_t<7>(c, B, stage, rows_all, nranks, m_total, m_total_dev)
                   : refine_stage_apply_t<6>(c, B, stage, rows_all, nranks, m_total, m_total_dev);
}

int refine_init_launch(Ctx* c, const RefineBuffers& B, int np) { return np == 7 ? refine_init_t<7>(c, B) : refine_init_t<6>(c, B); }
int refine_iter_launch(Ctx* c, const RefineBuffers& B, int np, int j, int chunk) { return np == 7 ? refine_iter_t<7>(c, B, j, chunk) : refine_iter_t<6>(c, B, j, chunk); }

int refine_finish_grid(const Ctx* c, const RefineBuffers& B) { return B.m_on_device ? refine_grid_cap(c) : refine_grid(c, B.m); }

int refine_finish_launch(Ctx* c, const RefineBuffers& B, double* inl_out) {
    if (!B.m_on_device && B.m == 0 && !B.zpartials && !B.state_host) return RSDSFM_OK;
    hipLaunchKernelGGL(refine_finish_kernel, dim3(refine_finish_grid(c, B)), dim3(kFB), 0, c->stream,
                       B.m_on_device ? (int64_t)-1 : B.m, B.inl, B.rho_a, B.rho_b, B.state, inl_out, B.zpartials, B.state_host, B.bad_index);
    RSDSFM_HIP_CHECK(c, hipGetLastError());
    return RSDSFM_OK;
}

}
```

### rs-aware-differential-sfm_amd/csrc/refine_rf_kernels.hip

```cpp
#include "refine_common.hpp"

#ifndef RF_LOADS_ONLY
#define RF_LOADS_ONLY 0
#endif
#ifndef RF_NP7_PREFETCH
#define RF_NP7_PREFETCH 0
#endif

namespace rsdsfm {

namespace {

constexpr int kRfListCap = 64;
constexpr int kRfEntry = 8;

template <int NP>
struct RfRow {
    static constexpr int TRI = NP * (NP + 1) / 2;
    static constexpr int OFF_JTJ = 0, OFF_B = TRI, OFF_JTB = 2 * TRI, OFF_C = 2 * TRI + NP;
    static constexpr int NSCHUR = 2 * TRI + 2 * NP;
    static constexpr int MODEL = NSCHUR, STEPSQ = NSCHUR + 1, COST2 = NSCHUR + 2, XSQ = NSCHUR + 3, ZSUM = NSCHUR + 4, GMAX = NSCHUR + 5;
    static constexpr int NW = NSCHUR + 6;
    static constexpr int NF = TRI + NP;
    static_assert(NW % 2 == 0, "rows are read as double2");
// ... 539 lines not shown
            st->solve_ok = rc == 1 ? 1 : 0;
            L.loop = again;
        }
        __syncthreads();
        RF_BEAT(21);
        const int again = L.loop;
        __syncthreads();
        if (!again) break;
        resolve = true;
    }
    RF_BEAT(30);
    if (ext_out) {
        if (tid < RR::NSCHUR) ext_out->sums[tid] = L.cur[tid];
        const int n = L.nlist;
        for (int q = tid; q < n * kRfEntry; q += kFB) ext_out->list[q] = L.list[q];
        if (tid == 0) ext_out->nlist = (double)n;
    }
    RF_BEAT(31);
#undef RF_BEAT
}

struct RfPassArgs {
    int64_t m;
    const double4* xyuv_in;
    double4* xyuv_out;
    double* beta;
    const double* alpha;
    const double* alpha_k;
    double* rho_a;
    double* rho_b;
    const RefineState* st_in;
    RefineState* st_out;
    const double* rows_prev;
    int nrows_prev, row_stride;
    RfLists lists_prev;
    int* list_count;
    double* list_entries;
    int* list_count_zero;
    const RfExt* ext_in;
    RfExt* ext_out;
    double* partials;
    double* trace;
    int trace_rows;
    int64_t m_total;
    const int64_t* m_total_dev;
    const double2* flow;
    int64_t n_flow;
    const double* inl;
    const int64_t* inlier_idx;
    int flow_index_mode;
    int* bad_index;
    unsigned long long* beat;
    int slot;
    unsigned long long* stamps;
};

struct RfLoad {
    double4 c4;
    double rho, ab, ak;
};
template <int NP>
__device__ __forceinline__ RfLoad rf_load(const RfPassArgs& A, const double* __restrict__ rho, int64_t i, bool live) {
    RfLoad l;
    l.c4 = make_double4(0.0, 0.0, 0.0, 0.0), l.rho = 0.0, l.ab = 0.0, l.ak = 0.0;
    if (live) {
        l.c4 = A.xyuv_in[i];
        l.rho = rho[i];
        if (NP == 6) {
            l.ab = A.beta[i];
        } else {
            l.ab = A.alpha[i], l.ak = A.alpha_k[i];
        }
    }
    return l;
}

}

template <int NP, bool FIRST, bool ZSUM>
__global__ __launch_bounds__(kFB) void refine_rf_pass_kernel(const RfPassArgs A) {
    using RR = RfRow<NP>;
    __shared__ RfStageLds<NP> s_stage;
    __shared__ double s_red[kFB / 64][RR::NW];
    __shared__ RefineState s_state;
    const bool stamp = A.stamps && blockIdx.x == 0 && threadIdx.x == 0;
    if (A.beat && threadIdx.x == 0) {
        if (A.beat[7]) atomicAdd(&A.beat[2], 1ull);
        if (blockIdx.x == 0) A.beat[0] = ((unsigned long long)A.slot << 8) | 1;
        if (blockIdx.x < 512) A.beat[8 + blockIdx.x] = ((unsigned long long)A.slot << 8) | 1;
    }
    __shared__ unsigned long long tk[8];
    if (stamp) {
#pragma unroll
        for (int i = 0; i < 8; ++i) tk[i] = 0;
    }
    if (stamp) tk[0] = wall_clock64();
    state_to_lds(&s_state, A.st_in);
    RefineState* st = &s_state;
    if (stamp) tk[1] = wall_clock64();
    if (FIRST) {
        if (threadIdx.x < 7) st->p0[threadIdx.x] = st->p[threadIdx.x];
        if (threadIdx.x == 0) st->rf = 1, st->rf_guard = 0, st->rf_resolves = 0, st->pending_apply = 0;
        __syncthreads();
    } else if (st->termination < 0 && st->pending_apply) {
        int64_t mt = A.m_total_dev ? *A.m_total_dev : (A.m_total >= 0 ? A.m_total : (A.m >= 0 ? A.m : st->m));
        rf_apply_body<NP>(st, s_stage, A.rows_prev, A.nrows_prev >= 0 ? A.nrows_prev : st->grid, A.row_stride, A.lists_prev, A.ext_in,
                          blockIdx.x == 0 ? A.ext_out : nullptr, mt, blockIdx.x == 0 ? A.trace : nullptr, A.trace_rows, stamp ? tk + 4 : nullptr);
        __syncthreads();
    }
    if (threadIdx.x == 0) st->pending_apply = st->termination < 0 ? 1 : 0;
    __syncthreads();
    if (stamp) tk[2] = wall_clock64();
    if (A.beat && threadIdx.x == 0) {
        if (blockIdx.x == 0) A.beat[0] = ((unsigned long long)A.slot << 8) | 2;
        if (blockIdx.x < 512) A.beat[8 + blockIdx.x] = ((unsigned long long)A.slot << 8) | ((st->termination >= 0 || (A.m < 0 && (int)blockIdx.x >= st->grid)) ? 9 : 2);
        if (A.beat[7] && (st->termination >= 0 || (A.m < 0 && (int)blockIdx.x >= st->grid))) atomicAdd(&A.beat[3], 1ull);
    }
    if (blockIdx.x == 0) {
        state_from_lds(A.st_out, st);
        if (threadIdx.x == 0) *A.list_count_zero = 0;
    }
    if (st->termination >= 0) return;
    const PassShape ps = pass_shape(st, A.m);
    if (!ps.live) return;
    const int64_t m = ps.m;
    double acc[RR::NW];
#pragma unroll
    for (int s = 0; s < RR::NW; ++s) acc[s] = 0.0;
    constexpr bool kLdsC = NP == 7 && !FIRST;
    __shared__ double s_cacc[kLdsC ? 3 * NP : 1][kLdsC ? kFB : 1];
    double* const lds_c = kLdsC ? &s_cacc[0][threadIdx.x] : nullptr;
    if (kLdsC) {
#pragma unroll
        for (int a = 0; a < 3 * NP; ++a) lds_c[a * kFB] = 0.0;
    }
    const int64_t stride = (int64_t)ps.grid * kFB;
    const int64_t i0 = (int64_t)blockIdx.x * kFB + threadIdx.x;
    RfPoint P0q = rf_point(st->p0);
    const RfPoint P0 = rf_point_uniform(P0q);
    if (FIRST) {
        RfPoint Pq = rf_point(st->p);
        const RfPoint P = rf_point_uniform(Pq);
        for (int64_t i = i0; i < m; i += stride) {
            int64_t fi = (A.flow_index_mode == RSDSFM_FLOW_GATHERED) ? A.inlier_idx[i] : i;
            if (fi < 0 || fi >= A.n_flow) {
                *A.bad_index = 1;
                fi = 0;
            }
            const double2 f = A.flow[fi];
            const double x = A.inl[3 * i], y = A.inl[3 * i + 1];
// ... 142 lines not shown
                                                             const RfExt* __restrict__ ext_in, RfExt* __restrict__ ext_out, int64_t m_total,
                                                             const int64_t* __restrict__ m_total_dev, double* __restrict__ trace, int trace_rows,
                                                             unsigned long long* __restrict__ beat, int slot) {
    __shared__ RfStageLds<NP> s_stage;
    __shared__ RefineState s_state;
    if (beat && threadIdx.x == 0) beat[1] = ((unsigned long long)slot << 8) | 1;
    state_to_lds(&s_state, st_in);
    RefineState* st = &s_state;
    if (st->termination < 0 && st->pending_apply) {
        const int64_t mt = m_total_dev ? *m_total_dev : (m_total >= 0 ? m_total : st->m);
        rf_apply_body<NP>(st, s_stage, rows, nrows >= 0 ? nrows : st->grid, row_stride, lists, ext_in, ext_out, mt, trace, trace_rows, nullptr, beat);
    }
    __syncthreads();
    if (beat && threadIdx.x == 0) beat[1] = ((unsigned long long)slot << 8) | 40;
    if (threadIdx.x == 0) st->pending_apply = 0;
    __syncthreads();
    state_from_lds(st_out, st);
}

template <int NP>
__global__ __launch_bounds__(kFB) void refine_rf_row_kernel(const double* __restrict__ partials, int nblocks, const RefineState* __restrict__ st,
                                                           const int* __restrict__ list_count, const double* __restrict__ list_entries,
                                                           double* __restrict__ row) {
    using RR = RfRow<NP>;
    __shared__ double s_grp[ReduceShape<RR::NW>::G][RR::NW];
    __shared__ double s[RR::NW];
    if (nblocks < 0) nblocks = st->grid;
    reduce_partials_groups<RR::NW>(partials, nblocks, RR::GMAX, s_grp, threadIdx.x, RR::NW, 0);
    __syncthreads();
    reduce_partials_slots<RR::NW>(s_grp, RR::GMAX, s, threadIdx.x);
    __syncthreads();
    if (threadIdx.x < RR::NW) row[threadIdx.x] = s[threadIdx.x];
    const int n = *list_count;
    double* lr = row + RR::NW;
    if (threadIdx.x == 0) {
        reinterpret_cast<int*>(lr)[0] = n;
        reinterpret_cast<int*>(lr)[1] = 0;
        lr[1] = 0.0;
    }
    if ((int)threadIdx.x < n && n <= kRfListCap) {
        const double* e = list_entries + (size_t)threadIdx.x * kRfEntry;
        int rank = 0;
        for (int j = 0; j < n; ++j) rank += (list_entries[(size_t)j * kRfEntry + 7] < e[7]) ? 1 : 0;
#pragma unroll
        for (int q = 0; q < kRfEntry; ++q) lr[2 + (size_t)rank * kRfEntry + q] = e[q];
    }
}


int refine_rf_extra_doubles() { return 3 * kRfListCap * kRfEntry + 2 * kRfExtDoubles + 8; }
int refine_rf_row_doubles(int np) { return (np == 7 ? RfRow<7>::NW : RfRow<6>::NW) + kRfListDoubles; }

namespace {
inline int rf_grid_cap(const Ctx* c) { return c->num_cus; }
inline int rf_grid(const Ctx* c, int64_t m) {
    int64_t b = (m + kFB - 1) / kFB;
    const int64_t cap = rf_grid_cap(c);
    if (b < 1) b = 1;
    if (b > cap) {
        const int64_t iters = (b + cap - 1) / cap;
        b = (b + iters - 1) / iters;
    }
    return (int)b;
}
struct RfLayout {
    double* rows[2];
    RefineState* cs[2];
    double* list[3];
    RfExt* ext[2];
};
inline RfLayout rf_layout(const Ctx* c, const RefineBuffers& B) {
    RfLayout Lo;
    double* base = B.partials;
    const size_t half = (size_t)refine_partials_half_doubles(c);
    Lo.rows[0] = base, Lo.rows[1] = base + half;
    double* p = base + 2 * half;
    const size_t sd = (size_t)refine_state_doubles();
    Lo.cs[0] = reinterpret_cast<RefineState*>(p), Lo.cs[1] = reinterpret_cast<RefineState*>(p + sd);
    p += 2 * sd + 8;
    for (int i = 0; i < 3; ++i) Lo.list[i] = p + (size_t)i * kRfListCap * kRfEntry;
    p += 3 * kRfListCap * kRfEntry;
    Lo.ext[0] = reinterpret_cast<RfExt*>(p), Lo.ext[1] = reinterpret_cast<RfExt*>(p + kRfExtDoubles);
    return Lo;
}
inline int rf_mod3(int g) { return ((g % 3) + 3) % 3; }
inline int* rf_list_count(const RefineBuffers& B, int g) { return refine_rf_counters(B) + rf_mod3(g); }
inline double* rf_list_entries(const RfLayout& Lo, int g) { return Lo.list[rf_mod3(g)]; }
inline RfLists rf_lists_of(const RfLayout& Lo, const RefineBuffers& B, int g, const double* rows_all, int nranks, int nw) {
    RfLists l;
    if (rows_all) {
        l.counts = reinterpret_cast<const int*>(rows_all + nw), l.count_stride = 2 * (nw + kRfListDoubles);
        l.entries = rows_all + nw + 2, l.entry_stride = nw + kRfListDoubles, l.nlists = nranks;
    } else {
        l.counts = rf_list_count(B, g), l.count_stride = 0, l.entries = rf_list_entries(Lo, g), l.entry_stride = 0, l.nlists = 1;
    }
    return l;
}

struct RfBeat {
    const Ctx* c;
    unsigned long long* words;
};
RfBeat g_beats[32];
int g_nbeats = 0;
unsigned long long* rf_beat(Ctx* c) {
    static const bool on = getenv("RSDSFM_SYNC_WATCHDOG_S") != nullptr && getenv("RSDSFM_NO_BEAT") == nullptr;
    if (!on) return nullptr;
    for (int i = 0; i < g_nbeats; ++i)
        if (g_beats[i].c == c) return g_beats[i].words;
    if (g_nbeats >= 32) return nullptr;
    unsigned long long* w = nullptr;
    if (hipHostMalloc((void**)&w, 64 + 8 * 512, hipHostMallocDefault) != hipSuccess) return nullptr;
    for (int i = 0; i < 8 + 512; ++i) w[i] = 0;
    w[7] = getenv("RSDSFM_BEAT_COUNT_WORKGROUPS") ? 1 : 0;
    g_beats[g_nbeats].c = c, g_beats[g_nbeats].words = w;
    ++g_nbeats;
    return w;
}
unsigned long long* rf_stamps(Ctx* c) {
    static int on = -1;
    static unsigned long long* buf = nullptr;
    if (on < 0) {
        const char* e = getenv("RSDSFM_RF_STAMPS");
        on = (e && e[0] == '1') ? 1 : 0;
        if (on && (hipMalloc(&buf, 128) != hipSuccess || hipMemset(buf, 0, 128) != hipSuccess)) buf = nullptr;
    }
    (void)c;
    return buf;
}
template <int NP, bool ZSUM>
void rf_pass_launch_t(Ctx* c, const RfPassArgs& A, bool first, int grid) {
    if (first)
        hipLaunchKernelGGL((refine_rf_pass_kernel<NP, true, ZSUM>), dim3(grid), dim3(kFB), 0, c->stream, A);
    else
        hipLaunchKernelGGL((refine_rf_pass_kernel<NP, false, ZSUM>), dim3(grid), dim3(kFB), 0, c->stream, A);
}
}

int refine_rf_pass_launch(Ctx* c, const RefineBuffers& B, int np, int g, int g_first, const double* rows_all_prev, int nranks, int64_t m_total,
                          const int64_t* m_total_dev, bool publish) {
    const RfLayout Lo = rf_layout(c, B);
    const int grid = B.m_on_device ? rf_grid_cap(c) : rf_grid(c, B.m);
    const int nw = np == 7 ? RfRow<7>::NW : RfRow<6>::NW;
    RfPassArgs A = {};
    A.m = B.m_on_device ? -1 : B.m;
    A.xyuv_in = reinterpret_cast<const double4*>(B.uu);
    A.xyuv_out = reinterpret_cast<double4*>(B.uu);
    A.beta = B.beta;
    A.alpha = B.alpha;
    A.alpha_k = B.alpha_k;
    A.rho_a = B.rho_a;
    A.rho_b = B.rho_b;
    A.st_in = g == g_first ? B.state : Lo.cs[(g - 1) & 1];
    A.st_out = publish ? B.state : Lo.cs[g & 1];
    if (rows_all_prev)
        A.rows_prev = rows_all_prev, A.nrows_prev = nranks, A.row_stride = nw + kRfListDoubles;
    else
        A.rows_prev = Lo.rows[(g - 1) & 1], A.nrows_prev = B.m_on_device ? -1 : grid, A.row_stride = nw;
    A.lists_prev = rf_lists_of(Lo, B, g - 1, rows_all_prev, nranks, nw);
    A.list_count = rf_list_count(B, g);
    A.list_entries = rf_list_entries(Lo, g);
    A.list_count_zero = rf_list_count(B, g + 1);
    A.ext_in = Lo.ext[(g - 1) & 1];
    A.ext_out = Lo.ext[g & 1];
    A.partials = Lo.rows[g & 1];
    A.trace = c->d_refine_trace;
    A.trace_rows = c->refine_trace_rows;
    A.m_total = m_total;
    A.m_total_dev = m_total_dev;
    A.flow = reinterpret_cast<const double2*>(B.flow);
    A.n_flow = B.n_flow;
    A.inl = B.inl;
    A.inlier_idx = B.inlier_idx;
    A.flow_index_mode = B.flow_index_mode;
    A.bad_index = B.bad_index;
    A.stamps = rf_stamps(c);
    A.beat = rf_beat(c);
    A.slot = g;
    const bool first = g == 0;
    if (np == 7) {
        if (B.want_zsum) rf_pass_launch_t<7, true>(c, A, first, grid); else rf_pass_launch_t<7, false>(c, A, first, grid);
    } else {
        if (B.want_zsum) rf_pass_launch_t<6, true>(c, A, first, grid); else rf_pass_launch_t<6, false>(c, A, first, grid);
    }
    RSDSFM_HIP_CHECK(c, hipGetLastError());
    return RSDSFM_OK;
}

int refine_rf_apply_launch(Ctx* c, const RefineBuffers& B, int np, int g, bool to_published, const double* rows_all, int nranks, int64_t m_total,
                           const int64_t* m_total_dev) {
    const RfLayout Lo = rf_layout(c, B);
    const int grid = B.m_on_device ? rf_grid_cap(c) : rf_grid(c, B.m);
    const int nw = np == 7 ? RfRow<7>::NW : RfRow<6>::NW;
    const double* rows = rows_all ? rows_all : Lo.rows[g & 1];
    const int nrows = rows_all ? nranks : (B.m_on_device ? -1 : grid);
    const int stride = rows_all ? nw + kRfListDoubles : nw;
    const RfLists lists = rf_lists_of(Lo, B, g, rows_all, nranks, nw);
    RefineState* st_io = Lo.cs[g & 1];
    if (np == 7)
        hipLaunchKernelGGL(refine_rf_apply_kernel<7>, dim3(1), dim3(kFB), 0, c->stream, rows, nrows, stride, lists, st_io, to_published ? B.state : st_io,
                           Lo.ext[g & 1], Lo.ext[(g + 1) & 1], m_total, m_total_dev, c->d_refine_trace, c->refine_trace_rows, rf_beat(c), g);
    else
        hipLaunchKernelGGL(refine_rf_apply_kernel<6>, dim3(1), dim3(kFB), 0, c->stream, rows, nrows, stride, lists, st_io, to_published ? B.state : st_io,
                           Lo.ext[g & 1], Lo.ext[(g + 1) & 1], m_total, m_total_dev, c->d_refine_trace, c->refine_trace_rows, rf_beat(c), g);
    RSDSFM_HIP_CHECK(c, hipGetLastError());
    return RSDSFM_OK;
}

int refine_rf_row_launch(Ctx* c, const RefineBuffers& B, int np, int g, double* row) {
    const RfLayout Lo = rf_layout(c, B);
    const int grid = B.m_on_device ? rf_grid_cap(c) : rf_grid(c, B.m);
    if (np == 7)
        hipLaunchKernelGGL(refine_rf_row_kernel<7>, dim3(1), dim3(kFB), 0, c->stream, Lo.rows[g & 1], B.m_on_device ? -1 : grid, static_cast<const RefineState*>(Lo.cs[g & 1]),
                           rf_list_count(B, g), rf_list_entries(Lo, g), row);
    else
        hipLaunchKernelGGL(refine_rf_row_kernel<6>, dim3(1), dim3(kFB), 0, c->stream, Lo.rows[g & 1], B.m_on_device ? -1 : grid, static_cast<const RefineState*>(Lo.cs[g & 1]),
                           rf_list_count(B, g), rf_list_entries(Lo, g), row);
    RSDSFM_HIP_CHECK(c, hipGetLastError());
    return RSDSFM_OK;
}

void refine_rf_debug_dump(Ctx* c, const RefineBuffers& B) {
    const RfLayout Lo = rf_layout(c, B);
    hipStream_t s2 = nullptr;
    if (hipStreamCreateWithFlags(&s2, hipStreamNonBlocking) != hipSuccess) return;
    RefineState h[3];
    int cnt[8] = {0, 0, 0, 0, 0, 0, 0, 0};
    const RefineState* src[3] = {B.state, Lo.cs[0], Lo.cs[1]};
// ... 42 lines not shown
```

### rs-aware-differential-sfm_amd/csrc/rsdsfm_internal.hpp

```cpp
#pragma once

#include <hip/hip_runtime.h>
#include <stdint.h>

#include <functional>
#include <string>
#include <vector>

#include "../../include/rsdsfm.h"

namespace rsdsfm {

constexpr int kMaxIter = 50;
constexpr int kRefineTraceCols = RSDSFM_REFINE_TRACE_COLS;
constexpr double kInitialRadius = 1e4;
constexpr double kMaxRadius = 1e16;
constexpr double kMinRadius = 1e-32;
constexpr double kMinRelDecrease = 1e-3;
constexpr double kMinLmDiag = 1e-6;
constexpr double kMaxLmDiag = 1e32;
constexpr double kFunctionTol = 1e-6;
constexpr double kGradientTol = 1e-10;
static_assert(kGradientTol < 1.0, "the indicator encoding of the gradient-maximum slots needs kGradientTol < 1");
constexpr double kParameterTol = 1e-8;
constexpr int kMaxInvalid = 5;
constexpr double kLmaTie = 1e-11;

constexpr int KMAX = 3;
constexpr int NS = 3 + 5 * KMAX;

struct Pose {
    double v[3];
    double w[3];
    double k;
};

struct LmScal {
    int32_t status;
    int32_t n_hist;
    int32_t K;
    int32_t write_which;
    int32_t iteration;
    int32_t num_successful;
    int32_t num_unsuccessful;
    int32_t invalid_run;
    int32_t termination;
    int32_t rho_holds;
    int32_t launches;
    int32_t next_launch;
    int32_t predict;
    int32_t restart;
    double radius;
    double decrease_factor;
    double cost;
    double initial_cost;
    double cand[KMAX];
};
struct LmState : LmScal {
    double hist[kMaxIter];
};

struct RansacBest {
    int32_t best_trial;
    int32_t undecided;
    int64_t num_inliers;
    int64_t num_inliers_scan;
    double inlier_error;
    double hyp[8];
    int32_t lma_tie;
    int32_t shared_best;
    int32_t _pad_shared;
    int32_t lazy_pending;
};
struct PickLazy {
    int* scored = nullptr;
    int* list = nullptr;
    int* list_count = nullptr;
};

constexpr int kScoreIdleLimit = 4;
constexpr int kRansacBatch = 128;

struct Ctx {
    int device = 0;
    hipStream_t stream = nullptr;
    bool own_stream = false;
    std::string err;
    double* d_partials = nullptr;
    unsigned* d_tickets = nullptr;
    LmState* d_lm = nullptr;
    LmState* h_lm = nullptr;
    int lm_issued_k = 0;
    int true_flow_exhaustive = 0;
    int ransac_fused_base = 2;
    int ransac_score_idle = kScoreIdleLimit;
    int refine_iters_hint = -1;
    int ransac_standard_math = 0;
    int* d_core_flag = nullptr;
    int core_epoch = 0;
    int ransac_math_mode = 0;
    int64_t ransac_restarts = 0;
    int lm_arithmetic = 0;
    int lma_hold = 0;
    bool lma_count_only_force = false;
    int64_t lma_count_only_runs = 0, lma_lazy_runs = 0;
    int lma_unique_run = 0;
    int64_t lma_restarts = 0;
    int64_t lma_handed_over = 0;
    int lma_last_guard = 0;
    int* d_lma_list = nullptr;
    int depth_lma_parity = 0;
    int lma_cand[2] = {2, 1};
    int ransac_spec_miss = 0;
    int frame_dense_hint = 1;
    int lm_issued_d = 0;
    int depth_epoch = 0;
    int depth_standard_math = 0;
    int64_t depth_restarts = 0;
    int depth_core_launch = 0;
    int prof_what = 0;
    void* d_stage = nullptr;
    size_t stage_bytes = 0;
    void* d_ws = nullptr;
    size_t ws_bytes = 0;
    void* d_frame = nullptr;
    size_t frame_bytes = 0;
    void* h_pinned = nullptr;
    hipEvent_t ev_ready = nullptr;
    size_t pinned_bytes = 0;
    int num_cus = 256;
    int ransac_k0 = 0;
    int ransac_not_one_step = -1;
    bool profile = false;
    hipEvent_t ev_prof[2] = {nullptr, nullptr};
    unsigned long long* d_clk_probe = nullptr;
    bool prof_pending = false;
    double* d_refine_trace = nullptr;
    int refine_trace_rows = 0;
    int depth_variant = 0;
    void* d_tile = nullptr;
    size_t tile_bytes = 0;
    void* tile_session = nullptr;
    int tile_np = 0;
    unsigned* d_claim[3] = {nullptr, nullptr, nullptr};
    size_t claim_words[3] = {0, 0, 0};
    unsigned claim_epoch[3] = {0, 0, 0};
    void* dist = nullptr;
    void* frame_run = nullptr;
    hipStream_t aux_stream = nullptr;
    hipEvent_t ev_fork = nullptr, ev_join = nullptr, ev_seq = nullptr;
    int frame_side_flatten = 3;
    unsigned long long* d_flat_counters = nullptr;
    int seq_lanes = 0;
    int refine_stage_mode = 0;
    bool refine_stage_separate = false;
    int refine_arithmetic = 0;
    int64_t refine_rf_runs = 0, refine_rf_restarts = 0, refine_rf_resolves = 0;
    int refine_rf_last_guard = 0;
    struct RansacCache {
        uint64_t tag = 0, stage_gen = 0;
        const double *d_u = nullptr, *d_inl = nullptr, *d_alpha = nullptr, *d_alpha_k = nullptr;
        const int64_t* d_idx = nullptr;
        int64_t n = 0, m = 0;
        const void* h_u = nullptr;
        double u_probe[16] = {0};
        double inl_probe[16] = {0};
    } ransac_cache;
    uint64_t stage_gen = 0, ransac_tag_counter = 0;
    int64_t refine_cache_hits = 0;
    std::vector<rsdsfm_ctx*> lanes;
};
constexpr int kSequenceLanesDefault = 3;
void dist_release(Ctx* c);
void dist_reset_hold(Ctx* c);
void frame_release(Ctx* c);

constexpr int kDepthBlock = 256;
constexpr int kDepthMaxBlocks = 512;
constexpr int kDecideBlock = 256;
constexpr int kDepthBatchMax = 8;

#define RSDSFM_HIP_CHECK(ctx, expr)                                                            \
    do {                                                                                       \
        hipError_t _e = (expr);                                                                \
        if (_e != hipSuccess) {                                                                \
            (ctx)->err = std::string(#expr) + ": " + hipGetErrorString(_e);                    \
            return RSDSFM_ERR_HIP;                                                             \
        }                                                                                      \
    } while (0)

struct DeviceGuard {
    int prev = -1;
    bool switched = false;
    explicit DeviceGuard(const Ctx* c) {
        if (hipGetDevice(&prev) == hipSuccess && prev != c->device) switched = hipSetDevice(c->device) == hipSuccess;
    }
    ~DeviceGuard() {
        if (switched) (void)hipSetDevice(prev);
    }
    DeviceGuard(const DeviceGuard&) = delete;
    DeviceGuard& operator=(const DeviceGuard&) = delete;
};

int fail(Ctx* c, int code, const char* msg);
// ... 81 lines not shown
int depth_map_launch(Ctx* c, double* d_inl, int64_t m, const double v[3], double fx, double fy, double cx, double cy, int rows,
                     int cols, double* d_depth_map, int32_t* d_xs, int32_t* d_ys, double* d_header, double* d_partials,
                     double* h_header = nullptr, const double* v_dev = nullptr, const int64_t* m_dev = nullptr,
                     const PoseTableOut* pt = nullptr);
int depth_map_slab_launch(Ctx* c, double* d_inl, int64_t m, const double* d_zsums, int nz, int64_t m_total, const double v[3],
                          double fx, double fy, double cx, double cy, int rows, int col0, int ncols, double* d_depth_map,
                          int32_t* d_xs, int32_t* d_ys, double* d_header, double* h_header = nullptr, const double* v_dev = nullptr,
                          const int64_t* m_dev = nullptr, const PoseTableOut* pt = nullptr);
int claim_map_acquire(Ctx* c, int which, size_t npix, unsigned** map, unsigned* tag, unsigned* mask);
int claim_map_reserve(Ctx* c, int which, size_t words);
int zsum_row_launch(Ctx* c, const double* d_inl, int64_t m, double* d_partials, double* d_out);
}

namespace rsdsfm {
struct Minimal9Direct {
    const double* img = nullptr;
    int rows = 0, cols = 0, alpha_ones = 0;
    double fx = 0, fy = 0, cx = 0, cy = 0, gamma = 0;
    int* core_flag = nullptr;
    int core_epoch = 0;
    double* probe = nullptr;
};
int minimal9_launch(Ctx* c, const double* q, const double* u, const double* alpha, const double* alpha_k,
                    const int32_t* samples, int T, int use_alpha_k, int k_sign_mode, double* hyp_out, void* zero_begin = nullptr,
                    size_t zero_bytes = 0, const Minimal9Direct* direct = nullptr);
struct DenseFlatten {
    double thr = 0.0;
    double *d_q = nullptr, *d_u = nullptr, *d_alpha = nullptr, *d_alpha_k = nullptr;
    unsigned long long* d_counters = nullptr;
    int64_t* total_out = nullptr;
};
int minimal9_flatten_launch(Ctx* c, const int32_t* samples, int T, int use_alpha_k, int k_sign_mode, double* hyp_out, void* zero_begin, size_t zero_bytes,
                            const Minimal9Direct& direct, double thr, double* d_q, double* d_u, double* d_alpha, double* d_alpha_k,
                            unsigned long long* d_counters, int64_t* total_out);
}

namespace rsdsfm {
int ransac_pixel_grid(const Ctx* c, int64_t n);
int ransac_lm_partials_doubles(const Ctx* c, int64_t n, int batch);
int ransac_lm_round_launch(Ctx* c, const double* q, const double* u, const double* a, const double* ak, int64_t n,
                           const double* hyp, int T, LmState* states, double* partials, int* flags, int* scored,
                           double* trial_count, double* trial_err, int round, double tol, int k0, int fused_base, bool core_math,
                           const int* m9_core_flag = nullptr, int m9_core_epoch = 0, int* unscored_list = nullptr);
int ransac_score_launch(Ctx* c, const double* q, const double* u, const double* a, const double* ak, int64_t n,
                        const double* hyp, int T, const LmState* states, int depth_mode, double tol, const int* scored,
                        double* partials, double* trial_count, double* trial_err, const int* unscored_list = nullptr, const int* unscored_count = nullptr);
int ransac_pick_launch(Ctx* c, const double* trial_count, const double* trial_err, int T, const double* hyp, RansacBest* best,
                       RansacBest* best_host = nullptr, const int* d_flags = nullptr, int* h_flags = nullptr, int scored_ahead = 0,
                       const double* cnt_rt = nullptr, int cnt_stride = 0, int nranks = 0, int64_t* m_all = nullptr, double tie_margin = 0.0,
                       PickLazy lazy = PickLazy());
int ransac_final_launch(Ctx* c, const double* q, const double* u, const double* a, const double* ak, int64_t n,
                        RansacBest* best, const LmState* states, int depth_mode, double tol, double* rho, uint8_t* mask,
                        int64_t* block_counts, int64_t* block_offsets, int64_t* inlier_idx, double* inliers,
                        double* out_alpha, double* out_alpha_k, RansacBest* best_host = nullptr);
int ransac_rows_doubles();
int ransac_lm_rows_launch(Ctx* c, const double* q, const double* u, const double* a, const double* ak, int64_t n,
                          const double* hyp, int T, const LmState* states, double* partials, int round, double tol, double* rows,
                          int* core_flags = nullptr, const int* m9_flag = nullptr, int m9_epoch = 0);
int ransac_rows_payload_doubles(int T, bool core_trailer);
int ransac_decide_rows_launch(Ctx* c, const double* rows_all, int nranks, int T, LmState* states, int64_t n_total, int round,
                              int* flags, int* scored, double* trial_count, double* trial_err, bool core_trailer = false,
                              double* cnt_rt = nullptr, int cnt_stride = 0);
int ransac_score_rows_launch(Ctx* c, const double* q, const double* u, const double* a, const double* ak, int64_t n,
                             const double* hyp, int T, const LmState* states, int depth_mode, double tol, const int* scored,
                             double* partials, double* rows);
int ransac_score_merge_launch(Ctx* c, const double* rows_all, int nranks, int T, const int* scored, double* trial_count,
                              double* trial_err, double* cnt_rt = nullptr, int cnt_stride = 0);
void sample_indices(int64_t n, int T, uint64_t seed, int32_t* out);
int64_t ransac_lma_partials_doubles(const Ctx* c, int64_t n, int batch);
size_t ransac_lma_list_ints(int batch);
int ransac_lma_launch(Ctx* c, const double* q, const double* u, const double* a, const double* ak, int64_t n, const double* hyp, int T,
                      LmState* states, double* partials, int* flags, int* scored, double* trial_count, double* trial_err, double tol,
                      const int* cand_steps, int ncand, int* irr_count, int* irr_list, int* unscored_list, int* guard_word,
                      const int* m9_core_flag = nullptr, int m9_core_epoch = 0, bool count_only = false);
int ransac_lma_rows_doubles();
int ransac_lma_rows_launch(Ctx* c, const double* q, const double* u, const double* a, const double* ak, int64_t n, const double* hyp, int T,
                           double* partials, double tol, const int* cand_steps, int ncand, int* irr_count, int* irr_list, double* rows);
int ransac_lma_decide_rows_launch(Ctx* c, const double* rows_all, int nranks, int64_t rank_stride, int T, int64_t n_total, const double* hyp,
                                  LmState* states, int* flags, int* scored, double* trial_count, double* trial_err, double tol, const int* cand_steps,
                                  int ncand, int* unscored_list, int* guard_word, double* cnt_rt, int cnt_stride, const int* m9_core_flag = nullptr,
                                  int m9_core_epoch = 0);
}

namespace rsdsfm {
struct RefineState {
    int32_t np, cur, iteration, invalid_run, num_successful, num_unsuccessful, termination, solve_ok;
    double p[7], pc[7], sp[7], yp[7];
    double radius, decrease_factor, cost, initial_cost, x_norm, gmax, stepsq_p;
    int64_t m;
    int32_t grid;
    int32_t need_schur;
    double zsum;
    int32_t slots;
    int32_t spec_miss_run;
    int32_t pending_apply;
    int32_t rf;
    double dp[7];
    double p0[7];
    int32_t rf_guard, rf_resolves;
};
constexpr int kTermRestartExact = 64;
struct RefineBuffers {
    const double* flow;
    int64_t n_flow, m;
    bool m_on_device = false;
    const double* inl;
    const double* alpha;
    const double* alpha_k;
    const int64_t* inlier_idx;
    int flow_index_mode;
    RefineState* state;
    double* uu;
    double* beta;
    double* rho_a;
    double* rho_b;
    double* srho;
    double* partials;
    int* bad_index;
    RefineState* state_host = nullptr;
    double* zpartials = nullptr;
    bool want_zsum = false;
};
size_t ransac_pinned_bytes(int T);
typedef std::function<int(const RansacBest*)> RansacSpecTail;
struct RansacRun {
    int pc = 0;
    const double *d_q = nullptr, *d_u = nullptr, *d_a = nullptr, *d_ak = nullptr;
    int64_t n = 0;
    int T = 0, Tn = 1, batch = 1, depth_mode = 0, use_alpha_k = 0, k_sign_mode = 0, k0 = 0, fused_base = 0;
    double tol = 0.0;
    rsdsfm_ransac_out* out = nullptr;
    const RansacSpecTail* spec_tail = nullptr;
    bool* spec_tail_held = nullptr;
    int core_epoch = 0;
    int* d_unscored = nullptr;
    bool core_math = true;
    bool analytic = false;
    bool lma_restarted = false;
    bool count_only = false;
    int lazy_rounds = 0;
    int shared_best = 0;
    double tie_margin = 0.0;
    int lma_guard = 0;
    bool lma_tie_seen = false;
    int lma_cand[2] = {2, 1}, lma_cand_next[2] = {0, 0};
    int *d_irr_count = nullptr, *d_irr_list = nullptr;
    bool restarted = false;
    bool tail_ahead = true;
    const Minimal9Direct* direct = nullptr;
    const DenseFlatten* dense = nullptr;
    const std::function<int()>* after_minimal9 = nullptr;
    std::vector<int32_t> samples;
    double *d_hyp = nullptr, *d_partials = nullptr, *d_tcount = nullptr, *d_terr = nullptr, *d_rho = nullptr;
    char* zero_begin = nullptr;
    size_t zero_bytes = 0;
    LmState* d_states = nullptr;
    int *d_scored = nullptr, *d_flags = nullptr;
    RansacBest* d_best = nullptr;
    int64_t *d_bcounts = nullptr, *d_boffs = nullptr;
    uint8_t* d_mask = nullptr;
    RansacBest* h_best = nullptr;
    int* h_running = nullptr;
    double *h_tcount = nullptr, *h_terr = nullptr, *h_hyp = nullptr;
    LmState* h_states = nullptr;
    int32_t* h_samples_pinned = nullptr;
    int b0 = 0, B = 0, round = 0;
    bool need_score = true, final_done = false, spec_scored = false, tail_enqueued = false, spec_final = false;
    int not_one_step = 0, fused_base_next = 0, score_hint_next = -1;
    bool hints_ready = false;
};
int ransac_begin(Ctx* c, const double* d_q, const double* d_u, const double* d_a, const double* d_ak, int64_t n, int use_alpha_k, int T,
                 double tol, const int32_t* h_samples, uint64_t seed, int depth_mode, int k_sign_mode, rsdsfm_ransac_out* out,
                 const RansacSpecTail* spec_tail, bool* spec_tail_held, RansacRun* run, const Minimal9Direct* direct,
                 const std::function<int()>* after_minimal9, const DenseFlatten* dense = nullptr, bool tail_ahead = true, bool count_only = false);
int ransac_finish(Ctx* c, RansacRun* run);
void ransac_commit_hints(Ctx* c, const RansacRun& run);
int flatten_enqueue(Ctx* c, const double* d_img, int32_t rows, int32_t cols, double fx, double fy, double cx, double cy, double gamma,
                    double thr, double* d_q, double* d_u, double* d_alpha, double* d_alpha_k, int64_t* h_total);
typedef std::function<int(const RefineBuffers&)> RefineTail;
int refine_finish_grid(const Ctx* c, const RefineBuffers& B);
struct RefineRun {
    RefineBuffers B;
    int np = 6, launched = 0, chunk = 5, hint_prev = -1;
    bool rf = false;
    double* d_inl_out = nullptr;
    const RefineTail* tail = nullptr;
    RefineState* hs = nullptr;
    bool prefetch = false, prefetched = false;
    bool tail_done = false;
};
constexpr size_t kPinnedTail = 1024;
size_t refine_workspace_bytes(const Ctx* c, int64_t m, bool m_on_device);
int refine_begin(Ctx* c, const double* d_flow, int64_t n_flow, int64_t m, const double* d_inl, const double* d_alpha,
                 const double* d_alpha_k, const int64_t* d_inlier_idx, const double v_in[3], const double w_in[3], double k_in,
                 int const_acceleration, int flow_index_mode, double* d_inl_out, const RefineTail* tail, const RansacBest* d_best,
                 void* ws_base, RefineRun* run, RefineState* hs_prefetch, double* d_zpartials, bool exact = false);
constexpr int kRcRefineRestartExact = 1;
int refine_device(Ctx* c, const double* d_flow, int64_t n_flow, int64_t m, const double* d_inl, const double* d_alpha,
                  const double* d_alpha_k, const int64_t* d_inlier_idx, const double v_in[3], const double w_in[3], double k_in,
                  int const_acceleration, int flow_index_mode, double* d_inl_out, double v_out[3], double w_out[3], double* k_out,
                  rsdsfm_lm_summary* summary, const RefineTail* tail, double* d_zpartials, bool exact = false);
int refine_enqueue_chunk(Ctx* c, RefineRun* run);
int frames_in_flight(const Ctx* c);
int refine_poll(Ctx* c, RefineRun* run, double v_out[3], double w_out[3], double* k_out, rsdsfm_lm_summary* summary);
int refine_partials_doubles(const Ctx* c, int64_t m);
int refine_partials_doubles_cap(const Ctx* c);
int refine_state_from_best_launch(Ctx* c, const RansacBest* d_best, const RefineBuffers& B, int np);
inline int refine_trace_reset(Ctx* c) {
    if (!c->d_refine_trace) return RSDSFM_OK;
    return hipMemsetAsync(c->d_refine_trace, 0xFF, (size_t)c->refine_trace_rows * kRefineTraceCols * sizeof(double), c->stream) == hipSuccess ? RSDSFM_OK : RSDSFM_ERR_HIP;
}
int refine_init_launch(Ctx* c, const RefineBuffers& B, int np);
int refine_rf_pass_launch(Ctx* c, const RefineBuffers& B, int np, int g, int g_first, const double* rows_all_prev, int nranks, int64_t m_total,
                          const int64_t* m_total_dev, bool publish = false);
int refine_rf_apply_launch(Ctx* c, const RefineBuffers& B, int np, int g, bool to_published, const double* rows_all, int nranks, int64_t m_total,
                           const int64_t* m_total_dev);
int refine_rf_row_launch(Ctx* c, const RefineBuffers& B, int np, int g, double* row);
int refine_rf_row_doubles(int np);
void refine_rf_debug_dump(Ctx* c, const RefineBuffers& B);
int refine_rf_read_stamps(Ctx* c, unsigned long long out[16]);
int refine_rf_extra_doubles();
int refine_partials_half_doubles(const Ctx* c);
int refine_state_doubles();
inline int* refine_rf_counters(const RefineBuffers& B) { return B.bad_index + 4; }
constexpr size_t kRefineStateBlockTail = 32;
int refine_iter_launch(Ctx* c, const RefineBuffers& B, int np, int j, int chunk);
int refine_finish_launch(Ctx* c, const RefineBuffers& B, double* inl_out);
int refine_stage_row_doubles(int np, int stage);
int refine_slot_row_doubles(int np);
int refine_slot_partials_doubles(const Ctx* c, int64_t m);
int refine_slot_rows_launch(Ctx* c, const RefineBuffers& B, int np, double* row, int j, const double* rows_all_prev, int nranks);
int refine_slot_apply_launch(Ctx* c, const RefineBuffers& B, int np, const double* rows_all, int nranks, int chunk);
int refine_stage_rows_launch(Ctx* c, const RefineBuffers& B, int np, int stage, double* row);
int refine_stage_apply_launch(Ctx* c, const RefineBuffers& B, int np, int stage, const double* rows_all, int nranks, int64_t m_total,
                              const int64_t* m_total_dev = nullptr);
}

namespace rsdsfm {
int back_project_launch(Ctx* c, const unsigned char* d_img, const double* d_depth_cm, const double* d_R, const double* d_t, double fx,
                        double fy, double cx, double cy, int rows, int cols, int mode, int q5_mode, unsigned char* d_gs, float* d_c3d);
int interpolate_cracky_launch(Ctx* c, const unsigned char* d_in, int rows, int cols, int offset, unsigned char* d_out);
int rectify_frame_launch(Ctx* c, const double* d_inl, int64_t m, const unsigned char* d_img, const double* d_depth_cm, const double* d_R,
                         const double* d_t, double fx, double fy, double cx, double cy, int rows, int cols, int mode, int q5_mode, int offset,
                         unsigned char* d_preview, unsigned char* d_gs, float* d_c3d, unsigned char* d_fixed, double* d_partials);
int depth_preview_launch(Ctx* c, const double* d_inl, int64_t m, double fx, double fy, double cx, double cy, int rows, int cols,
                         unsigned char* d_out, double* d_partials);
}

struct rsdsfm_ctx {
    rsdsfm::Ctx c;
};
```

Before: 1697.

## Shorten frame tail by folding state init, flag zeroing and depth write into launches

Adds a default-on frame tail mode that cuts several small launches at the end of a frame. The refine first pass now builds its starting state directly from the RANSAC best result. The RANSAC scatter kernel zeroes the refine flag words itself, replacing a separate memset. A new depth_decide_write kernel reduces the z-sum partials, decides the sign flip and writes the depth map from per-pixel owner tags, replacing the slab depth-map path. The aim is to remove launch and serialization overhead in the tail, at the cost of more coupling between stages and reliance on an owner-claim buffer being filled correctly.

```diff
diff --git a/include/rsdsfm.h b/include/rsdsfm.h
--- a/include/rsdsfm.h
+++ b/include/rsdsfm.h
@@ -186,6 +186,7 @@
                             rsdsfm_frame_result* results);
 int rsdsfm_set_sequence_lanes(rsdsfm_ctx* ctx, int32_t lanes);
 int rsdsfm_set_frame_side_flatten(rsdsfm_ctx* ctx, int mode);
+int rsdsfm_set_frame_tail(rsdsfm_ctx* ctx, int mode);
 int rsdsfm_ransac_dev(rsdsfm_ctx* ctx, const double* d_q2n, const double* d_u2n, const double* d_alpha_n,
                       const double* d_alpha_k_n, int64_t n, int use_alpha_k, int32_t iterations, double tolerance,
                       const int32_t* samples_9xT_or_null, uint64_t seed, int depth_mode, int k_sign_mode,
diff --git a/rs-aware-differential-sfm_amd/__init__.py b/rs-aware-differential-sfm_amd/__init__.py
--- a/rs-aware-differential-sfm_amd/__init__.py
+++ b/rs-aware-differential-sfm_amd/__init__.py
@@ -515,6 +515,9 @@
     def set_frame_side_flatten(self, on):
         self._check(self.lib.rsdsfm_set_frame_side_flatten(self._ctx, int(on)), "rsdsfm_set_frame_side_flatten")
 
+    def set_frame_tail(self, mode):
+        self._check(self.lib.rsdsfm_set_frame_tail(self._ctx, int(mode)), "rsdsfm_set_frame_tail")
+
     def prepared_frames_solve(self, jobs, trials=50, tol=0.05, use_acceleration_mode=False, use_refinement=True, depth_mode=DEPTH_CERES_LM,
                               k_sign_mode=K_COMPAT, flow_threshold=1e-10, flow_index_mode=FLOW_COMPAT_RANK, use_global_shutter_mode=False):
         n = len(jobs)
diff --git a/rs-aware-differential-sfm_amd/csrc/frame_host.hip b/rs-aware-differential-sfm_amd/csrc/frame_host.hip
--- a/rs-aware-differential-sfm_amd/csrc/frame_host.hip
+++ b/rs-aware-differential-sfm_amd/csrc/frame_host.hip
@@ -38,6 +38,7 @@
     int rc_begin = RSDSFM_OK;
     int64_t m_known = -1;
     RefineTail tail;
+    FinishClaim claim;
     RansacSpecTail spec_tail;
     std::function<int()> join;
 };
@@ -200,12 +201,23 @@
         PoseTableOut pt;
         if (J2.d_R_rows9_or_null && J2.d_t_rows3_or_null)
             pt.R = J2.d_R_rows9_or_null, pt.t = J2.d_t_rows3_or_null, pt.rows = J2.rows, pt.gamma = J2.gamma, pt.wk_dev = st->p + 3;
+        if (B.claim.on)
+            return depth_map_decided_launch(c, F->d_inl_ref, m_arg, F->d_zpartials, refine_finish_grid(c, B), B, J2.d_depth_map_colmajor, F->d_zheader,
+                                            header_host(c), st->p, m_dev, &pt);
         return depth_map_slab_launch(c, F->d_inl_ref, m_arg, F->d_zpartials, refine_finish_grid(c, B), m_arg, nullptr, J2.fx, J2.fy, J2.cx, J2.cy, J2.rows,
                                      0, J2.cols, J2.d_depth_map_colmajor, nullptr, F->d_ys, F->d_zheader, header_host(c), st->p, m_dev, &pt);
     };
+    F->claim = FinishClaim();
+    if (c->frame_tail == 0) {
+        F->claim.on = true;
+        F->claim.fx = J.fx, F->claim.fy = J.fy, F->claim.cx = J.cx, F->claim.cy = J.cy;
+        F->claim.rows = rows, F->claim.cols = cols;
+        F->claim.ys = F->d_ys;
+    }
     F->spec_tail = [c, F](const RansacBest* d_best) -> int {
         return refine_begin(c, F->d_u, F->n, F->n, F->d_inl, F->d_in_a, F->d_in_ak, F->d_idx, nullptr, nullptr, 0.0, F->prm.use_acceleration_mode,
-                            F->prm.flow_index_mode, F->d_inl_ref, &F->tail, d_best, F->d_refine_ws, &F->refine, state_host(c), F->d_zpartials);
+                            F->prm.flow_index_mode, F->d_inl_ref, &F->tail, d_best, F->d_refine_ws, &F->refine, state_host(c), F->d_zpartials, false,
+                            &F->claim);
     };
     F->refinement_enqueued = false;
     F->ahead = prm->use_refinement && c->ransac_spec_miss < 2;
@@ -215,7 +227,8 @@
     F->rc_begin = ransac_begin(c, F->d_q, F->d_u, F->d_a, F->d_ak, n, prm->use_acceleration_mode, prm->ransac_trials, prm->ransac_tol, nullptr, J.seed,
                                prm->depth_mode, prm->k_sign_mode, &F->ro, prm->use_refinement ? &F->spec_tail : nullptr, &F->refinement_enqueued, &F->ransac,
                                F->side_flatten ? &F->direct : nullptr, F->side_flatten && !F->dense_in_launch ? &F->join : nullptr,
-                               F->dense_in_launch ? &F->dense : nullptr, F->ahead, true);
+                               F->dense_in_launch ? &F->dense : nullptr, F->ahead, true,
+                               F->claim.on && prm->use_refinement ? refine_flag_words(F->d_refine_ws) : nullptr);
     return RSDSFM_OK;
 }
 
@@ -250,7 +263,8 @@
         counted = false;
         rc = ransac_begin(c, F->d_q, F->d_u, F->d_a, F->d_ak, n, prm->use_acceleration_mode, prm->ransac_trials, prm->ransac_tol, nullptr, J.seed,
                           prm->depth_mode, prm->k_sign_mode, &F->ro, prm->use_refinement ? &F->spec_tail : nullptr, &F->refinement_enqueued, &F->ransac, nullptr, nullptr,
-                          nullptr, F->ahead, true);
+                          nullptr, F->ahead, true,
+                               F->claim.on && prm->use_refinement ? refine_flag_words(F->d_refine_ws) : nullptr);
         if (rc == RSDSFM_OK) rc = ransac_finish(c, &F->ransac);
         counted = rc == RSDSFM_OK;
     }
@@ -277,7 +291,7 @@
         }
         if (!F->refinement_enqueued || exact)
             rc = refine_device(c, F->d_u, n, ro.num_inliers, F->d_inl, F->d_in_a, F->d_in_ak, F->d_idx, v, w, k, prm->use_acceleration_mode,
-                               prm->flow_index_mode, F->d_inl_ref, v, w, &k, &res->refine_summary, &F->tail, F->d_zpartials, exact);
+                               prm->flow_index_mode, F->d_inl_ref, v, w, &k, &res->refine_summary, &F->tail, F->d_zpartials, exact, &F->claim);
         if (rc != RSDSFM_OK) return rc;
         d_final = F->d_inl_ref;
         const double* h_header = header_host(c);
@@ -368,6 +382,13 @@
     return RSDSFM_OK;
 }
 
+int rsdsfm_set_frame_tail(rsdsfm_ctx* ctx, int mode) {
+    if (!ctx) return RSDSFM_ERR_INVALID;
+    if (mode < 0 || mode > 1) return fail(&ctx->c, RSDSFM_ERR_INVALID, "mode must be 0 (short launch tail) or 1 (stage-by-stage launches)");
+    ctx->c.frame_tail = mode;
+    return RSDSFM_OK;
+}
+
 int rsdsfm_set_frame_side_flatten(rsdsfm_ctx* ctx, int mode) {
     if (!ctx) return RSDSFM_ERR_INVALID;
     if (mode < 0 || mode > 3) return fail(&ctx->c, RSDSFM_ERR_INVALID, "mode must be 0 (flatten first), 1 (flatten on a second stream), 2 (flatten behind the minimal solver) or 3 (flatten inside the solver's launch)");
@@ -402,6 +423,7 @@
         lc->refine_arithmetic = c->refine_arithmetic;
         lc->lma_count_only_force = c->lma_count_only_force;
         lc->frame_side_flatten = c->frame_side_flatten;
+        lc->frame_tail = c->frame_tail;
         lc->refine_stage_mode = c->refine_stage_mode;
     }
     for (int l = 0; l < L; ++l) lane_ctx(l)->refine_stage_separate = L > 1;
diff --git a/rs-aware-differential-sfm_amd/csrc/glue_kernels.hip b/rs-aware-differential-sfm_amd/csrc/glue_kernels.hip
--- a/rs-aware-differential-sfm_amd/csrc/glue_kernels.hip
+++ b/rs-aware-differential-sfm_amd/csrc/glue_kernels.hip
@@ -240,6 +240,55 @@
     }
 }
 
+__global__ __launch_bounds__(kGB) void depth_decide_write_kernel(const double* __restrict__ partials, int nblocks, int64_t m, double* __restrict__ header,
+                                                                double* __restrict__ header_host, const double* __restrict__ v_dev,
+                                                                const int64_t* __restrict__ m_dev, PoseTableOut pt, double* __restrict__ inl,
+                                                                const double* __restrict__ rho_a, const double* __restrict__ rho_b,
+                                                                const RefineState* __restrict__ st, const unsigned* __restrict__ owner, unsigned tag,
+                                                                unsigned mask, int64_t npix, double* __restrict__ depth_map) {
+    static_assert(kGB == 256, "zsum_decide_kernel's reduction shape");
+    __shared__ double s_red[4];
+    if (m_dev) m = *m_dev;
+    double acc = 0.0;
+    for (int b = threadIdx.x; b < nblocks; b += 256) acc += partials[b];
+    const double r = wave_sum(acc);
+    if ((threadIdx.x & 63) == 0) s_red[threadIdx.x >> 6] = r;
+    __syncthreads();
+    const double count_z = ((s_red[0] + s_red[1]) + s_red[2]) + s_red[3];
+    const double z_mean = count_z * 1.0 / (double)m;
+    const bool flip = z_mean < 0;
+    Pose pose;
+    pose.v[0] = flip ? v_dev[0] * -1.0 : v_dev[0];
+    pose.v[1] = flip ? v_dev[1] * -1.0 : v_dev[1];
+    pose.v[2] = flip ? v_dev[2] * -1.0 : v_dev[2];
+    if (blockIdx.x == 0 && threadIdx.x == 0) {
+        header[0] = flip ? 1.0 : 0.0;
+        header[1] = pose.v[0], header[2] = pose.v[1], header[3] = pose.v[2];
+        if (header_host) {
+            header_host[0] = flip ? 1.0 : 0.0;
+            header_host[1] = pose.v[0], header_host[2] = pose.v[1], header_host[3] = pose.v[2];
+        }
+    }
+    const int64_t stride = (int64_t)gridDim.x * kGB;
+    const int64_t g0 = (int64_t)blockIdx.x * kGB + threadIdx.x;
+    if (pt.R) {
+        pose.w[0] = pt.wk_dev[0], pose.w[1] = pt.wk_dev[1], pose.w[2] = pt.wk_dev[2], pose.k = pt.wk_dev[3];
+        for (int64_t i = g0; i < pt.rows; i += stride) pose_table_row(pose, pt.gamma, pt.rows, (int)i, pt.R, pt.t);
+    }
+    const double* __restrict__ rho = st->cur ? rho_b : rho_a;
+    for (int64_t p = g0; p < npix; p += stride) {
+        const unsigned w = owner[p];
+        double d = 0.0;
+        if ((w & ~mask) == tag) {
+            const double z = 1.0 / rho[(int64_t)(w & mask)];
+            d = flip ? z * -1.0 : z;
+        }
+        depth_map[p] = d;
+    }
+    if (flip)
+        for (int64_t i = g0; i < m; i += stride) inl[3 * i + 2] = inl[3 * i + 2] * -1.0;
+}
+
 constexpr int kScanSeg = kScanSegCells;
 
 __global__ __launch_bounds__(256) void cell_scan_local_kernel(const int64_t* __restrict__ counts, int64_t ncells,
@@ -396,6 +445,17 @@
     return RSDSFM_OK;
 }
 
+int depth_map_decided_launch(Ctx* c, double* d_inl, int64_t m, const double* d_zsums, int nz, const RefineBuffers& B, double* d_depth_map,
+                             double* d_header, double* h_header, const double* v_dev, const int64_t* m_dev, const PoseTableOut* pt) {
+    const FinishClaim& C = B.claim;
+    if (!C.on || !C.owner || !v_dev) return fail(c, RSDSFM_ERR_INVALID, "depth map: no output pass has claimed the pixels");
+    const int64_t npix = (int64_t)C.rows * C.cols;
+    hipLaunchKernelGGL(depth_decide_write_kernel, dim3(stream_grid(npix)), dim3(kGB), 0, c->stream, d_zsums, nz, m, d_header, h_header, v_dev, m_dev,
+                       pt ? *pt : PoseTableOut(), d_inl, B.rho_a, B.rho_b, B.state, C.owner, C.tag, C.mask, npix, d_depth_map);
+    RSDSFM_HIP_CHECK(c, hipGetLastError());
+    return RSDSFM_OK;
+}
+
 int depth_map_launch(Ctx* c, double* d_inl, int64_t m, const double v[3], double fx, double fy, double cx, double cy, int rows,
                      int cols, double* d_depth_map, int32_t* d_xs, int32_t* d_ys, double* d_header, double* d_partials,
                      double* h_header, const double* v_dev, const int64_t* m_dev, const PoseTableOut* pt) {
diff --git a/rs-aware-differential-sfm_amd/csrc/ransac_host.hip b/rs-aware-differential-sfm_amd/csrc/ransac_host.hip
--- a/rs-aware-differential-sfm_amd/csrc/ransac_host.hip
+++ b/rs-aware-differential-sfm_amd/csrc/ransac_host.hip
@@ -182,7 +182,7 @@
                     if (rc != RSDSFM_OK) return rc;
                     flags_via_pick = true;
                     rc = ransac_final_launch(c, R.d_q, R.d_u, R.d_a, R.d_ak, n, R.d_best, R.d_states, depth_mode, tol, R.d_rho, R.d_mask, R.d_bcounts,
-                                             R.d_boffs, out->inlier_idx, out->inliers, out->alpha, out->alpha_k, R.h_best);
+                                             R.d_boffs, out->inlier_idx, out->inliers, out->alpha, out->alpha_k, R.h_best, R.refine_flag_words);
                     if (rc != RSDSFM_OK) return rc;
                     R.final_done = true;
                     R.spec_final = true;
@@ -269,7 +269,7 @@
                                             R.count_only ? PickLazy{R.d_scored, R.d_unscored, R.d_flags + 1} : PickLazy());
                     if (rc != RSDSFM_OK) return rc;
                     rc = ransac_final_launch(c, R.d_q, R.d_u, R.d_a, R.d_ak, n, R.d_best, R.d_states, depth_mode, tol, R.d_rho, R.d_mask, R.d_bcounts,
-                                             R.d_boffs, out->inlier_idx, out->inliers, out->alpha, out->alpha_k, R.h_best);
+                                             R.d_boffs, out->inlier_idx, out->inliers, out->alpha, out->alpha_k, R.h_best, R.refine_flag_words);
                     if (rc != RSDSFM_OK) return rc;
                 }
                 if (R.spec_tail && !R.tail_enqueued) {
@@ -371,7 +371,7 @@
 int ransac_begin(Ctx* c, const double* d_q, const double* d_u, const double* d_a, const double* d_ak, int64_t n, int use_alpha_k, int T,
                  double tol, const int32_t* h_samples, uint64_t seed, int depth_mode, int k_sign_mode, rsdsfm_ransac_out* out,
                  const RansacSpecTail* spec_tail, bool* spec_tail_held, RansacRun* run, const Minimal9Direct* direct,
-                 const std::function<int()>* after_minimal9, const DenseFlatten* dense, bool tail_ahead, bool count_only) {
+                 const std::function<int()>* after_minimal9, const DenseFlatten* dense, bool tail_ahead, bool count_only, int* refine_flag_words) {
     RansacRun& R = *run;
     R = RansacRun();
     R.tail_ahead = tail_ahead;
@@ -381,6 +381,7 @@
     R.lma_cand[0] = c->lma_cand[0], R.lma_cand[1] = c->lma_cand[1];
     R.count_only = count_only && R.analytic && T <= kRansacBatch && (c->lma_unique_run >= 2 || c->lma_count_only_force);
     if (R.count_only) R.tie_margin = 0.0;
+    R.refine_flag_words = refine_flag_words;
     if (spec_tail_held) *spec_tail_held = false;
     if (!out) return fail(c, RSDSFM_ERR_INVALID, "null out");
     if (n < 9) return fail(c, RSDSFM_ERR_INVALID, "ransac needs at least 9 points (the reference would compute rand() % 0)");
diff --git a/rs-aware-differential-sfm_amd/csrc/ransac_kernels.hip b/rs-aware-differential-sfm_amd/csrc/ransac_kernels.hip
--- a/rs-aware-differential-sfm_amd/csrc/ransac_kernels.hip
+++ b/rs-aware-differential-sfm_amd/csrc/ransac_kernels.hip
@@ -789,9 +789,11 @@
                                                             const double* __restrict__ rho, const uint8_t* __restrict__ mask,
                                                             const int64_t* __restrict__ block_counts, RansacBest* best,
                                                             RansacBest* best_host, int64_t* __restrict__ inlier_idx, double* __restrict__ inliers,
-                                                            double* __restrict__ out_alpha, double* __restrict__ out_alpha_k) {
+                                                            double* __restrict__ out_alpha, double* __restrict__ out_alpha_k,
+                                                            int* __restrict__ zero_words = nullptr) {
     __shared__ int s_wave[kRB / 64];
     __shared__ int64_t s_base;
+    if (zero_words && blockIdx.x == 0 && threadIdx.x < (int)(kRefineStateBlockTail / sizeof(int))) zero_words[threadIdx.x] = 0;
     __shared__ int64_t s_pre[kRB / 64], s_all[kRB / 64];
     const int tid = threadIdx.x, lane = tid & 63, wv = tid >> 6;
     const int undecided = best->undecided;
@@ -1017,7 +1019,7 @@
 int ransac_final_launch(Ctx* c, const double* q, const double* u, const double* a, const double* ak, int64_t n,
                         RansacBest* best, const LmState* states, int depth_mode, double tol, double* rho, uint8_t* mask,
                         int64_t* block_counts, int64_t* block_offsets, int64_t* inlier_idx, double* inliers,
-                        double* out_alpha, double* out_alpha_k, RansacBest* best_host) {
+                        double* out_alpha, double* out_alpha_k, RansacBest* best_host, int* zero_words) {
     int64_t blocks = (n + kRB - 1) / kRB;
     if (blocks < 1) blocks = 1;
     const int64_t cap = 2048;
@@ -1032,8 +1034,9 @@
     RSDSFM_HIP_CHECK(c, hipGetLastError());
     if (inlier_idx || inliers || out_alpha || out_alpha_k) {
         hipLaunchKernelGGL(ransac_scatter_kernel, dim3((int)blocks), dim3(kRB), 0, c->stream, reinterpret_cast<const double2*>(q),
-                           a, ak, n, chunk, rho, mask, block_counts, best, best_host, inlier_idx, inliers, out_alpha, out_alpha_k);
+                           a, ak, n, chunk, rho, mask, block_counts, best, best_host, inlier_idx, inliers, out_alpha, out_alpha_k, zero_words);
     } else {
+        if (zero_words) RSDSFM_HIP_CHECK(c, hipMemsetAsync(zero_words, 0, kRefineStateBlockTail, c->stream));
         hipLaunchKernelGGL(ransac_scan_kernel, dim3(1), dim3(256), 0, c->stream, block_counts, (int)blocks, block_offsets, best, best_host);
     }
     RSDSFM_HIP_CHECK(c, hipGetLastError());
diff --git a/rs-aware-differential-sfm_amd/csrc/refine_host.hip b/rs-aware-differential-sfm_amd/csrc/refine_host.hip
--- a/rs-aware-differential-sfm_amd/csrc/refine_host.hip
+++ b/rs-aware-differential-sfm_amd/csrc/refine_host.hip
@@ -9,7 +9,7 @@
 int refine_begin(Ctx* c, const double* d_flow, int64_t n_flow, int64_t m, const double* d_inl, const double* d_alpha,
                  const double* d_alpha_k, const int64_t* d_inlier_idx, const double v_in[3], const double w_in[3], double k_in,
                  int const_acceleration, int flow_index_mode, double* d_inl_out, const RefineTail* tail, const RansacBest* d_best,
-                 void* ws_base, RefineRun* run, RefineState* hs_prefetch, double* d_zpartials, bool exact) {
+                 void* ws_base, RefineRun* run, RefineState* hs_prefetch, double* d_zpartials, bool exact, const FinishClaim* claim) {
     if (m < 0 || n_flow < 0 || (!d_best && (!v_in || !w_in))) return fail(c, RSDSFM_ERR_INVALID, "bad arguments");
     if (flow_index_mode != RSDSFM_FLOW_COMPAT_RANK && flow_index_mode != RSDSFM_FLOW_GATHERED) return fail(c, RSDSFM_ERR_INVALID, "unknown flow_index_mode");
     if (flow_index_mode == RSDSFM_FLOW_GATHERED && m > 0 && !d_inlier_idx) return fail(c, RSDSFM_ERR_INVALID, "gathered mode needs inlier_idx");
@@ -48,6 +48,7 @@
     B.partials = ws.take<double>(npart);
     B.bad_index = reinterpret_cast<int*>(state_block + sizeof(RefineState));
     B.zpartials = d_zpartials;
+    if (claim && claim->on && d_zpartials) B.claim = *claim;
     run->np = np;
     run->rf = !exact && c->lm_arithmetic == 0 && c->refine_arithmetic == 0;
     if (run->rf) c->refine_rf_runs += 1;
@@ -59,7 +60,9 @@
     run->prefetch = hs_prefetch != nullptr;
     run->prefetched = false;
     B.state_host = hs_prefetch;
-    if (d_best) {
+    if (d_best && claim && claim->on && run->rf && !c->refine_stage_separate) {
+        B.best_dev = d_best;
+    } else if (d_best) {
         rc = refine_state_from_best_launch(c, d_best, B, np);
         if (rc != RSDSFM_OK) return rc;
     } else {
@@ -113,7 +116,15 @@
         }
     }
     run->launched += run->chunk;
-    int rc = refine_finish_launch(c, run->B, run->d_inl_out);
+    int rc = RSDSFM_OK;
+    if (run->B.claim.on) {
+        FinishClaim& C = run->B.claim;
+        const int64_t npix = (int64_t)C.rows * C.cols;
+        if (run->B.m >= ((int64_t)1 << 31)) return fail(c, RSDSFM_ERR_INVALID, "depth map: more than 2^31 inliers");
+        rc = claim_map_acquire(c, 2, (size_t)std::max<int64_t>(std::max<int64_t>(npix, run->B.m), 1), &C.owner, &C.tag, &C.mask);
+        if (rc != RSDSFM_OK) return rc;
+    }
+    rc = refine_finish_launch(c, run->B, run->d_inl_out);
     if (rc != RSDSFM_OK) return rc;
     run->tail_done = false;
     if (run->tail && !(run->hint_prev > run->launched + 1)) {
@@ -173,6 +184,11 @@
     return RSDSFM_OK;
 }
 
+int* refine_flag_words(void* ws_base) {
+    Arena ws(ws_base);
+    return reinterpret_cast<int*>(ws.take<char>(sizeof(RefineState) + 64) + sizeof(RefineState));
+}
+
 size_t refine_workspace_bytes(const Ctx* c, int64_t m, bool m_on_device) {
     const size_t M = (size_t)std::max<int64_t>(m, 1);
     const size_t npart = (size_t)(m_on_device ? refine_partials_doubles_cap(c) : refine_partials_doubles(c, m));
@@ -182,13 +198,13 @@
 int refine_device(Ctx* c, const double* d_flow, int64_t n_flow, int64_t m, const double* d_inl, const double* d_alpha,
                   const double* d_alpha_k, const int64_t* d_inlier_idx, const double v_in[3], const double w_in[3], double k_in,
                   int const_acceleration, int flow_index_mode, double* d_inl_out, double v_out[3], double w_out[3], double* k_out,
-                  rsdsfm_lm_summary* summary, const RefineTail* tail, double* d_zpartials, bool exact) {
+                  rsdsfm_lm_summary* summary, const RefineTail* tail, double* d_zpartials, bool exact, const FinishClaim* claim) {
     if (!v_out || !w_out || !k_out) return fail(c, RSDSFM_ERR_INVALID, "bad arguments");
     const double v0[3] = {v_in[0], v_in[1], v_in[2]}, w0[3] = {w_in[0], w_in[1], w_in[2]};
     for (int attempt = 0;; ++attempt) {
         RefineRun run;
         int rc = refine_begin(c, d_flow, n_flow, m, d_inl, d_alpha, d_alpha_k, d_inlier_idx, v0, w0, k_in, const_acceleration, flow_index_mode,
-                              d_inl_out, tail, nullptr, nullptr, &run, nullptr, d_zpartials, exact || attempt > 0);
+                              d_inl_out, tail, nullptr, nullptr, &run, nullptr, d_zpartials, exact || attempt > 0, claim);
         if (rc != RSDSFM_OK) return rc;
         rc = refine_poll(c, &run, v_out, w_out, k_out, summary);
         if (rc != kRcRefineRestartExact || attempt > 0) return rc == kRcRefineRestartExact ? fail(c, RSDSFM_ERR_NUMERIC, "refinement: restart loop") : rc;
diff --git a/rs-aware-differential-sfm_amd/csrc/refine_kernels.hip b/rs-aware-differential-sfm_amd/csrc/refine_kernels.hip
--- a/rs-aware-differential-sfm_amd/csrc/refine_kernels.hip
+++ b/rs-aware-differential-sfm_amd/csrc/refine_kernels.hip
@@ -454,6 +454,44 @@
             for (int w2 = 1; w2 < kFB / 64; ++w2) t += s_red[w2];
             zpartials[blockIdx.x] = t;
         }
+    }
+}
+
+__global__ __launch_bounds__(kFB) void refine_finish_claim_kernel(int64_t m, const double* __restrict__ inl, const double* __restrict__ rho_a,
+                                                                 const double* __restrict__ rho_b, const RefineState* __restrict__ st,
+                                                                 double* __restrict__ inl_out, double* __restrict__ zpartials,
+                                                                 RefineState* __restrict__ state_host, const int* __restrict__ bad_index,
+                                                                 double fx, double fy, double cx, double cy, int rows, int ncols,
+                                                                 unsigned* __restrict__ owner, unsigned tag, int32_t* __restrict__ ys) {
+    __shared__ double s_red[kFB / 64];
+    if (state_host && blockIdx.x == 0) {
+        for (int i = threadIdx.x; i < (int)(sizeof(RefineState) / 8); i += kFB)
+            reinterpret_cast<double*>(state_host)[i] = reinterpret_cast<const double*>(st)[i];
+        if (threadIdx.x == 0) *reinterpret_cast<int*>(reinterpret_cast<char*>(state_host) + sizeof(RefineState)) = *bad_index;
+    }
+    const double* __restrict__ rho = st->cur ? rho_b : rho_a;
+    if (m < 0) m = st->m;
+    const int64_t stride = (int64_t)gridDim.x * kFB;
+    double acc = 0.0;
+    for (int64_t i = (int64_t)blockIdx.x * kFB + threadIdx.x; i < m; i += stride) {
+        const double xn = inl[3 * i], yn = inl[3 * i + 1];
+        inl_out[3 * i] = xn;
+        inl_out[3 * i + 1] = yn;
+        const double z = 1.0 / rho[i];
+        inl_out[3 * i + 2] = z;
+        acc += z;
+        const int x = (int)(fx * xn + cx + 0.5);
+        const int y = (int)(fy * yn + cy + 0.5);
+        ys[i] = y;
+        if (x >= 0 && x < ncols && y >= 0 && y < rows) atomicMax(&owner[(int64_t)x * rows + y], tag | (unsigned)i);
+    }
+    const double r = wave_sum(acc);
+    if ((threadIdx.x & 63) == 0) s_red[threadIdx.x >> 6] = r;
+    __syncthreads();
+    if (threadIdx.x == 0) {
+        double t = s_red[0];
+        for (int w2 = 1; w2 < kFB / 64; ++w2) t += s_red[w2];
+        zpartials[blockIdx.x] = t;
     }
 }
 
@@ -857,6 +895,13 @@
 
 int refine_finish_launch(Ctx* c, const RefineBuffers& B, double* inl_out) {
     if (!B.m_on_device && B.m == 0 && !B.zpartials && !B.state_host) return RSDSFM_OK;
+    if (B.claim.on) {
+        hipLaunchKernelGGL(refine_finish_claim_kernel, dim3(refine_finish_grid(c, B)), dim3(kFB), 0, c->stream, B.m_on_device ? (int64_t)-1 : B.m, B.inl,
+                           B.rho_a, B.rho_b, B.state, inl_out, B.zpartials, B.state_host, B.bad_index, B.claim.fx, B.claim.fy, B.claim.cx, B.claim.cy,
+                           B.claim.rows, B.claim.cols, B.claim.owner, B.claim.tag, B.claim.ys);
+        RSDSFM_HIP_CHECK(c, hipGetLastError());
+        return RSDSFM_OK;
+    }
     hipLaunchKernelGGL(refine_finish_kernel, dim3(refine_finish_grid(c, B)), dim3(kFB), 0, c->stream,
                        B.m_on_device ? (int64_t)-1 : B.m, B.inl, B.rho_a, B.rho_b, B.state, inl_out, B.zpartials, B.state_host, B.bad_index);
     RSDSFM_HIP_CHECK(c, hipGetLastError());
diff --git a/rs-aware-differential-sfm_amd/csrc/refine_rf_kernels.hip b/rs-aware-differential-sfm_amd/csrc/refine_rf_kernels.hip
--- a/rs-aware-differential-sfm_amd/csrc/refine_rf_kernels.hip
+++ b/rs-aware-differential-sfm_amd/csrc/refine_rf_kernels.hip
@@ -615,6 +615,8 @@
     int* bad_index;
     unsigned long long* beat;
     int slot;
+    const RansacBest* best;
+    int grid_cap;
     unsigned long long* stamps;
 };
 
@@ -658,7 +660,34 @@
         for (int i = 0; i < 8; ++i) tk[i] = 0;
     }
     if (stamp) tk[0] = wall_clock64();
-    state_to_lds(&s_state, A.st_in);
+    if (FIRST && A.best) {
+        if (threadIdx.x < sizeof(RefineState) / 8) reinterpret_cast<unsigned long long*>(&s_state)[threadIdx.x] = 0ull;
+        __syncthreads();
+        if (threadIdx.x == 0) {
+            RefineState& z = s_state;
+            z.np = NP;
+            for (int i = 0; i < 3; ++i) {
+                z.p[i] = A.best->hyp[3 + i];
+                z.p[3 + i] = A.best->hyp[i];
+            }
+            z.p[6] = A.best->hyp[6];
+            z.termination = -1;
+            z.radius = kInitialRadius;
+            z.need_schur = 1;
+            const int64_t mb = A.best->undecided ? 0 : A.best->num_inliers_scan;
+            z.m = mb;
+            int64_t b = (mb + kFB - 1) / kFB;
+            if (b < 1) b = 1;
+            if (b > A.grid_cap) {
+                const int64_t iters = (b + A.grid_cap - 1) / A.grid_cap;
+                b = (b + iters - 1) / iters;
+            }
+            z.grid = (int)b;
+        }
+        __syncthreads();
+    } else {
+        state_to_lds(&s_state, A.st_in);
+    }
     RefineState* st = &s_state;
     if (stamp) tk[1] = wall_clock64();
     if (FIRST) {
@@ -907,6 +936,7 @@
 int refine_rf_row_doubles(int np) { return (np == 7 ? RfRow<7>::NW : RfRow<6>::NW) + kRfListDoubles; }
 
 namespace {
+static_assert(kWorkgroupsPerCu == 1, "rf_grid_cap and the cap of RefineState::grid (refine_state_from_best_kernel) agree only at one workgroup per CU");
 inline int rf_grid_cap(const Ctx* c) { return c->num_cus; }
 inline int rf_grid(const Ctx* c, int64_t m) {
     int64_t b = (m + kFB - 1) / kFB;
@@ -924,6 +954,7 @@
     double* list[3];
     RfExt* ext[2];
 };
+static_assert(RfRow<7>::NW <= SlotRow<7>::NW && RfRow<6>::NW <= SlotRow<7>::NW, "the rows buffer is sized by SlotRow<7>::NW doubles per workgroup");
 inline RfLayout rf_layout(const Ctx* c, const RefineBuffers& B) {
     RfLayout Lo;
     double* base = B.partials;
@@ -1029,6 +1060,8 @@
     A.inlier_idx = B.inlier_idx;
     A.flow_index_mode = B.flow_index_mode;
     A.bad_index = B.bad_index;
+    A.best = g == 0 ? B.best_dev : nullptr;
+    A.grid_cap = rf_grid_cap(c);
     A.stamps = rf_stamps(c);
     A.beat = rf_beat(c);
     A.slot = g;
diff --git a/rs-aware-differential-sfm_amd/csrc/rsdsfm_internal.hpp b/rs-aware-differential-sfm_amd/csrc/rsdsfm_internal.hpp
--- a/rs-aware-differential-sfm_amd/csrc/rsdsfm_internal.hpp
+++ b/rs-aware-differential-sfm_amd/csrc/rsdsfm_internal.hpp
@@ -60,6 +60,7 @@
     double hist[kMaxIter];
 };
 
+constexpr size_t kRefineStateBlockTail = 32;
 struct RansacBest {
     int32_t best_trial;
     int32_t undecided;
@@ -150,6 +151,7 @@
     hipStream_t aux_stream = nullptr;
     hipEvent_t ev_fork = nullptr, ev_join = nullptr, ev_seq = nullptr;
     int frame_side_flatten = 3;
+    int frame_tail = 0;
     unsigned long long* d_flat_counters = nullptr;
     int seq_lanes = 0;
     int refine_stage_mode = 0;
@@ -337,7 +339,7 @@
 int ransac_final_launch(Ctx* c, const double* q, const double* u, const double* a, const double* ak, int64_t n,
                         RansacBest* best, const LmState* states, int depth_mode, double tol, double* rho, uint8_t* mask,
                         int64_t* block_counts, int64_t* block_offsets, int64_t* inlier_idx, double* inliers,
-                        double* out_alpha, double* out_alpha_k, RansacBest* best_host = nullptr);
+                        double* out_alpha, double* out_alpha_k, RansacBest* best_host = nullptr, int* zero_words = nullptr);
 int ransac_rows_doubles();
 int ransac_lm_rows_launch(Ctx* c, const double* q, const double* u, const double* a, const double* ak, int64_t n,
                           const double* hyp, int T, const LmState* states, double* partials, int round, double tol, double* rows,
@@ -385,6 +387,14 @@
     int32_t rf_guard, rf_resolves;
 };
 constexpr int kTermRestartExact = 64;
+struct FinishClaim {
+    bool on = false;
+    double fx = 0.0, fy = 0.0, cx = 0.0, cy = 0.0;
+    int rows = 0, cols = 0;
+    int32_t* ys = nullptr;
+    unsigned* owner = nullptr;
+    unsigned tag = 0, mask = 0;
+};
 struct RefineBuffers {
     const double* flow;
     int64_t n_flow, m;
@@ -404,6 +414,8 @@
     int* bad_index;
     RefineState* state_host = nullptr;
     double* zpartials = nullptr;
+    const RansacBest* best_dev = nullptr;
+    FinishClaim claim;
     bool want_zsum = false;
 };
 size_t ransac_pinned_bytes(int T);
@@ -422,6 +434,7 @@
     bool core_math = true;
     bool analytic = false;
     bool lma_restarted = false;
+    int* refine_flag_words = nullptr;
     bool count_only = false;
     int lazy_rounds = 0;
     int shared_best = 0;
@@ -457,13 +470,16 @@
 int ransac_begin(Ctx* c, const double* d_q, const double* d_u, const double* d_a, const double* d_ak, int64_t n, int use_alpha_k, int T,
                  double tol, const int32_t* h_samples, uint64_t seed, int depth_mode, int k_sign_mode, rsdsfm_ransac_out* out,
                  const RansacSpecTail* spec_tail, bool* spec_tail_held, RansacRun* run, const Minimal9Direct* direct,
-                 const std::function<int()>* after_minimal9, const DenseFlatten* dense = nullptr, bool tail_ahead = true, bool count_only = false);
+                 const std::function<int()>* after_minimal9, const DenseFlatten* dense = nullptr, bool tail_ahead = true, bool count_only = false,
+                 int* refine_flag_words = nullptr);
 int ransac_finish(Ctx* c, RansacRun* run);
 void ransac_commit_hints(Ctx* c, const RansacRun& run);
 int flatten_enqueue(Ctx* c, const double* d_img, int32_t rows, int32_t cols, double fx, double fy, double cx, double cy, double gamma,
                     double thr, double* d_q, double* d_u, double* d_alpha, double* d_alpha_k, int64_t* h_total);
 typedef std::function<int(const RefineBuffers&)> RefineTail;
 int refine_finish_grid(const Ctx* c, const RefineBuffers& B);
+int depth_map_decided_launch(Ctx* c, double* d_inl, int64_t m, const double* d_zsums, int nz, const RefineBuffers& B, double* d_depth_map,
+                             double* d_header, double* h_header, const double* v_dev, const int64_t* m_dev, const PoseTableOut* pt);
 struct RefineRun {
     RefineBuffers B;
     int np = 6, launched = 0, chunk = 5, hint_prev = -1;
@@ -479,18 +495,20 @@
 int refine_begin(Ctx* c, const double* d_flow, int64_t n_flow, int64_t m, const double* d_inl, const double* d_alpha,
                  const double* d_alpha_k, const int64_t* d_inlier_idx, const double v_in[3], const double w_in[3], double k_in,
                  int const_acceleration, int flow_index_mode, double* d_inl_out, const RefineTail* tail, const RansacBest* d_best,
-                 void* ws_base, RefineRun* run, RefineState* hs_prefetch, double* d_zpartials, bool exact = false);
+                 void* ws_base, RefineRun* run, RefineState* hs_prefetch, double* d_zpartials, bool exact = false,
+                 const FinishClaim* claim = nullptr);
 constexpr int kRcRefineRestartExact = 1;
 int refine_device(Ctx* c, const double* d_flow, int64_t n_flow, int64_t m, const double* d_inl, const double* d_alpha,
                   const double* d_alpha_k, const int64_t* d_inlier_idx, const double v_in[3], const double w_in[3], double k_in,
                   int const_acceleration, int flow_index_mode, double* d_inl_out, double v_out[3], double w_out[3], double* k_out,
-                  rsdsfm_lm_summary* summary, const RefineTail* tail, double* d_zpartials, bool exact = false);
+                  rsdsfm_lm_summary* summary, const RefineTail* tail, double* d_zpartials, bool exact = false, const FinishClaim* claim = nullptr);
 int refine_enqueue_chunk(Ctx* c, RefineRun* run);
 int frames_in_flight(const Ctx* c);
 int refine_poll(Ctx* c, RefineRun* run, double v_out[3], double w_out[3], double* k_out, rsdsfm_lm_summary* summary);
 int refine_partials_doubles(const Ctx* c, int64_t m);
 int refine_partials_doubles_cap(const Ctx* c);
 int refine_state_from_best_launch(Ctx* c, const RansacBest* d_best, const RefineBuffers& B, int np);
+int* refine_flag_words(void* ws_base);
 inline int refine_trace_reset(Ctx* c) {
     if (!c->d_refine_trace) return RSDSFM_OK;
     return hipMemsetAsync(c->d_refine_trace, 0xFF, (size_t)c->refine_trace_rows * kRefineTraceCols * sizeof(double), c->stream) == hipSuccess ? RSDSFM_OK : RSDSFM_ERR_HIP;
@@ -508,7 +526,6 @@
 int refine_partials_half_doubles(const Ctx* c);
 int refine_state_doubles();
 inline int* refine_rf_counters(const RefineBuffers& B) { return B.bad_index + 4; }
-constexpr size_t kRefineStateBlockTail = 32;
 int refine_iter_launch(Ctx* c, const RefineBuffers& B, int np, int j, int chunk);
 int refine_finish_launch(Ctx* c, const RefineBuffers& B, double* inl_out);
 int refine_stage_row_doubles(int np, int stage);
```

Measured after the change: 1735, median of 6. 2.2% higher.
